# roryclear/clearcam

Measured on AMD Instinct MI355X. Metric: yolov9c_640x640_frames_per_sec, higher is better.
Workload: dtype f16; 1 GPU; YOLOv9-C f16h batch=64 640x640 frames (letterbox 640) per GPU, uint8 BGR frames resident in HBM, seeded synthetic weights, full detect path (letterbox+convs+decode+top300+NMS); batch_per_gpu=64, parallelism=one camera batch per GPU x1, no collective, batches_in_flight=3

## Files before the change

### clearcam_amd/_lib.py

```python
from __future__ import annotations

import ctypes as C
import os

_HERE = os.path.dirname(os.path.abspath(__file__))
LIB_PATH = os.path.join(_HERE, "libclearcam_hip.so")

SYMBOLS = [
    "cc_last_error", "cc_version", "cc_device_count",
    "cc_yolo_create", "cc_yolo_load", "cc_yolo_calibrate", "cc_yolo_calibration_info", "cc_gptq_round_f16", "cc_yolo_finalize", "cc_yolo_detect", "cc_yolo_set_in_flight", "cc_yolo_submit", "cc_yolo_wait",
    "cc_yolo_detect_ragged", "cc_yolo_submit_ragged", "cc_letterbox_geometry", "cc_yolo_plans_built",
    "cc_yolo_get_tensor", "cc_yolo_get_tensor_frames", "cc_yolo_nonfinite",
    "cc_yolo_last_gpu_ms", "cc_yolo_profile", "cc_yolo_profile_graph", "cc_yolo_destroy", "cc_conv2d_nhwc", "cc_conv2d_ex", "cc_route_log_take", "cc_conv_bench", "cc_dev_set", "cc_round_weights", "cc_attn_bench",
    "cc_dev_decode", "cc_dev_head_tail", "cc_dev_topk_nms", "cc_dev_blaze_post",
    "cc_dev_pool", "cc_dev_pool_choice", "cc_dev_fuse", "cc_dev_conv_src", "cc_dev_affine", "cc_dev_face_pre",
    "cc_dev_csp", "cc_dev_csp_choice", "cc_dev_stem",
    "cc_dev_attention", "cc_dev_layernorm", "cc_dev_assemble_ln", "cc_dev_patchify", "cc_dev_embed", "cc_dev_l2norm",
    "cc_clip_create", "cc_clip_load", "cc_clip_finalize", "cc_clip_encode_image", "cc_clip_encode_text",
    "cc_clip_set_in_flight", "cc_clip_submit_image", "cc_clip_wait",
    "cc_clip_last_gpu_ms", "cc_clip_destroy", "cc_crop_preprocess", "cc_cv_resize_linear_u8", "cc_cv_warp_affine_u8",
    "cc_blaze_create", "cc_blaze_load", "cc_blaze_finalize", "cc_blaze_detect", "cc_blaze_detect_batch", "cc_blaze_destroy",
    "cc_face_locate", "cc_face_align",
    "cc_face_create", "cc_face_load", "cc_face_finalize", "cc_face_embed", "cc_face_destroy",
    "cc_ocsort_create", "cc_ocsort_update", "cc_ocsort_update_many", "cc_ocsort_num_tracks", "cc_ocsort_destroy",
    "cc_index_create", "cc_index_create_ex", "cc_index_add", "cc_index_add_grouped", "cc_index_size", "cc_index_info", "cc_index_scores", "cc_index_last_path",
    "cc_index_search", "cc_index_search_groups", "cc_index_add_tracked", "cc_index_search_tracks", "cc_index_rank",
    "cc_index_add_described", "cc_index_row_info", "cc_index_rank_where", "cc_index_timeline", "cc_index_fetch_rows", "cc_index_rank_like",
    "cc_index_rank_terms", "cc_index_timeline_terms",
    "cc_index_gram", "cc_index_distinct", "cc_index_digest", "cc_index_sightings",
    "cc_index_remove_rows", "cc_index_remove_groups", "cc_index_destroy",
    "cc_watch_create", "cc_watch_set", "cc_watch_size", "cc_watch_scores", "cc_watch_match", "cc_watch_destroy",
]


class ClipConfig(C.Structure):
    _fields_ = [(n, C.c_int) for n in ("image_size", "patch", "v_width", "v_layers", "v_heads", "v_mlp",
                                       "t_ctx", "t_vocab", "t_width", "t_layers", "t_heads", "t_mlp", "embed")]


class ConvDesc(C.Structure):
    _fields_ = [(n, C.c_int) for n in ("dtype", "B", "H", "W", "Cin", "Cout", "k", "stride", "groups", "act", "pad", "Ho", "Wo",
                                       "out_f32", "out_cstride", "out_coff", "res_f32", "res_cstride", "res_coff", "variant")]


class SrcDesc(C.Structure):
    _fields_ = [("ptr", C.c_void_p)] + [(n, C.c_int) for n in ("H", "W", "cstride", "coff", "C", "shift")]


DEV_CSP_LAYERS = 3
DEV_CONV_ADOWN = 100
ROUTE_REC_INTS = 18


class FaceAlignRec(C.Structure):
    _fields_ = [("offset", C.c_int64), ("h", C.c_int32), ("w", C.c_int32),
                ("cx1", C.c_int32), ("cy1", C.c_int32), ("cw", C.c_int32), ("ch", C.c_int32),
                ("out_w", C.c_int32), ("out_h", C.c_int32), ("rot", C.c_double * 6), ("place", C.c_double * 6)]


ROW_NO_TS = -(1 << 31)
RANK_TRACKS = 1
LIKE_MAX_ROWS = 64
LIKE_EXCLUDE_ROWS, LIKE_EXCLUDE_TRACK = 2, 4
TERMS_MAX = 64
TERM_RANK, TERM_REQUIRE, TERM_REJECT = 0, 1, 2
COMBINE_MAX, COMBINE_MIN, COMBINE_SUM = 0, 1, 2
DISTINCT_MAX_DEPTH, DISTINCT_MAX_Q = 1024, 64
DIGEST_MAX_LEADERS = 1024
DIGEST_BY_COUNT, DIGEST_BY_FIRST = 0, 1
SIGHT_MAX_OBJECTS, SIGHT_MAX_GROUPS = 1024, 4096
SIGHT_SKIP_SELF = 1


class RowFilter(C.Structure):
    _fields_ = [("use_ts", C.c_int32), ("ts_min", C.c_int32), ("ts_max", C.c_int32), ("use_cls", C.c_int32), ("cls_mask", C.c_uint64 * 4)]


class Term(C.Structure):
    _fields_ = [("role", C.c_int32), ("weight", C.c_float), ("cut", C.c_float)]


class CCError(RuntimeError):
    pass


_lib = None


def lib() -> C.CDLL:
    global _lib
    if _lib is not None:
        return _lib
    if not os.path.exists(LIB_PATH):
        raise CCError(f"{LIB_PATH} not built: run `python -c 'import __graft_entry__ as g; g.build()'` "
                      "(hipcc --offload-arch=gfx950). There is no CPU fallback.")
    try:
        import torch
    except ImportError:
        pass
    L = C.CDLL(LIB_PATH)
    L.cc_last_error.restype = C.c_char_p
    vp, ip, fp, i64p = C.c_void_p, C.POINTER(C.c_int), C.POINTER(C.c_float), C.POINTER(C.c_int64)
    sig = {
        "cc_version": [],
        "cc_device_count": [ip],
        "cc_yolo_create": [C.POINTER(vp), C.c_char_p, C.c_int, C.c_int, C.c_int],
        "cc_yolo_load": [vp, C.c_char_p, vp, i64p, C.c_int],
        "cc_yolo_finalize": [vp],
        "cc_yolo_calibrate": [vp, vp, C.c_int, C.c_int, C.c_int, C.c_int],
        "cc_yolo_calibration_info": [vp, ip, ip],
        "cc_gptq_round_f16": [vp, C.c_int64, C.c_int64, vp, C.c_double, vp],
        "cc_yolo_detect": [vp, vp, C.c_int, C.c_int, C.c_int, C.c_int, C.c_int, vp, C.c_int, vp],
        "cc_yolo_set_in_flight": [vp, C.c_int],
        "cc_yolo_submit": [vp, vp, C.c_int, C.c_int, C.c_int, C.c_int, C.c_int, vp, C.c_int, vp, C.POINTER(C.c_longlong)],
        "cc_yolo_wait": [vp, C.c_longlong, vp],
        "cc_yolo_detect_ragged": [vp, vp, i64p, C.POINTER(C.c_int32), C.POINTER(C.c_int32), C.c_int, C.c_int, C.c_int, vp, C.c_int, vp],
        "cc_yolo_submit_ragged": [vp, vp, i64p, C.POINTER(C.c_int32), C.POINTER(C.c_int32), C.c_int, C.c_int, C.c_int, vp, C.c_int, vp, C.POINTER(C.c_longlong)],
        "cc_letterbox_geometry": [C.c_int, C.c_int, C.c_int, ip, ip, ip, ip],
        "cc_yolo_plans_built": [vp, ip],
        "cc_yolo_get_tensor": [vp, C.c_char_p, vp, i64p, ip],
        "cc_yolo_get_tensor_frames": [vp, C.c_char_p, C.c_int, C.c_int, vp, i64p, ip],
        "cc_yolo_nonfinite": [vp, ip],
        "cc_yolo_last_gpu_ms": [vp, fp],
        "cc_yolo_profile": [vp, C.c_int, fp, C.POINTER(C.c_double), ip],
        "cc_yolo_profile_graph": [vp, C.c_int, C.c_int, fp],
        "cc_conv2d_nhwc": [C.c_int, vp, C.c_int, C.c_int, C.c_int, C.c_int, vp, vp, C.c_int, C.c_int, C.c_int, C.c_int,
                           C.c_int, vp, C.c_int, vp],
        "cc_conv2d_ex": [C.POINTER(ConvDesc), vp, vp, vp, vp, vp, vp, ip, vp],
        "cc_route_log_take": [ip, C.c_int, ip],
        "cc_dev_decode": [vp, ip, ip, C.c_int, vp, C.c_float, vp, ip, vp],
        "cc_dev_head_tail": [C.c_int, C.c_int, vp, vp, vp, vp, vp, vp, ip, ip, C.c_int, vp, C.c_float, vp, ip, vp],
        "cc_dev_topk_nms": [vp, C.c_int, C.c_int, C.c_float, vp, C.c_int, vp, vp],
        "cc_dev_blaze_post": [vp, vp, vp, vp, C.c_int, vp, C.c_float, C.c_int, C.c_int, vp, vp, vp, vp],
        "cc_dev_pool": [C.c_int, vp, C.c_int, C.c_int, vp] + [C.c_int] * 12 + [ip, vp],
        "cc_dev_pool_choice": [C.c_int, vp, C.c_int, C.c_int, vp] + [C.c_int] * 12 + [ip],
        "cc_dev_fuse": [C.c_int, C.c_int, vp, ip, ip, ip, ip, ip, vp, C.c_int, C.c_int, C.c_int, C.c_int, C.c_int, C.c_int, vp],
        "cc_dev_conv_src": [C.POINTER(ConvDesc), C.POINTER(SrcDesc), C.POINTER(SrcDesc), vp, vp, vp, ip, vp],
        "cc_dev_affine": [C.c_int, vp, vp, vp, vp, C.c_longlong, C.c_int, vp],
        "cc_dev_face_pre": [C.c_int, vp, C.c_int, vp, C.c_int, C.c_int, vp],
        "cc_dev_csp": [C.c_int, C.c_int, C.c_int, vp, C.c_int, C.c_int, vp, C.c_int, C.c_int, C.c_int, C.c_int, C.c_int, C.POINTER(vp), C.POINTER(vp),
                       C.c_int, C.c_int, ip, vp],
        "cc_dev_csp_choice": [C.c_int] * 8 + [ip],
        "cc_dev_stem": [C.c_int, C.c_int, vp, C.c_int, i64p, C.POINTER(C.c_int32), C.POINTER(C.c_int32), C.c_int, C.c_int, C.c_int, vp, vp, C.c_int,
                        vp, C.c_int, C.c_int, ip, vp],
        "cc_dev_attention": [C.c_int, vp, C.c_int, C.c_int, C.c_int, C.c_int, C.c_float, vp, vp],
        "cc_dev_layernorm": [C.c_int, vp, C.c_longlong, vp, vp, vp, vp, C.c_int, C.c_int, C.c_int, vp],
        "cc_dev_assemble_ln": [C.c_int, vp, vp, vp, vp, vp, vp, C.c_int, C.c_int, C.c_int, vp],
        "cc_dev_patchify": [C.c_int, vp, vp, C.c_int, C.c_int, C.c_int, C.c_int, vp],
        "cc_dev_embed": [vp, C.c_int, vp, vp, vp, C.c_int, C.c_int, C.c_int, vp],
        "cc_dev_l2norm": [vp, C.c_int, C.c_int, C.c_float, vp],
        "cc_conv_bench": [C.c_int] * 11 + [fp],
        "cc_dev_set": [C.c_char_p, C.c_int],
        "cc_round_weights": [C.c_int, vp, C.c_int64, C.c_int64, C.c_int64, vp],
        "cc_attn_bench": [C.c_int] * 7 + [fp],
        "cc_clip_create": [C.POINTER(vp), C.POINTER(ClipConfig), C.c_int, C.c_int],
        "cc_clip_load": [vp, C.c_char_p, vp, i64p, C.c_int],
        "cc_clip_finalize": [vp],
        "cc_clip_encode_image": [vp, vp, C.c_int, C.c_int, vp, C.c_int, vp],
        "cc_clip_encode_text": [vp, vp, C.c_int, vp, C.c_int, vp],
        "cc_clip_set_in_flight": [vp, C.c_int],
        "cc_clip_submit_image": [vp, vp, C.c_int, C.c_int, vp, C.c_int, vp, C.POINTER(C.c_longlong)],
        "cc_clip_wait": [vp, C.c_longlong, vp],
        "cc_clip_last_gpu_ms": [vp, fp],
        "cc_crop_preprocess": [vp, vp, vp, vp, C.c_int, C.c_int, C.c_int, vp, C.c_int, vp],
        "cc_cv_resize_linear_u8": [vp, C.c_int, C.c_int, vp, C.c_int, C.c_int, C.c_int],
        "cc_cv_warp_affine_u8": [vp, C.c_int, C.c_int, vp, vp, C.c_int, C.c_int, C.c_int],
        "cc_blaze_create": [C.POINTER(vp), C.c_int, C.c_int],
        "cc_blaze_load": [vp, C.c_char_p, vp, i64p, C.c_int],
        "cc_blaze_finalize": [vp],
        "cc_blaze_detect": [vp, vp, C.c_int, C.c_int, C.c_int, C.c_int, vp, C.c_int, vp],
        "cc_blaze_detect_batch": [vp, vp, C.c_int, C.c_int, C.c_int, C.c_int, C.c_int, vp, C.c_int, vp],
        "cc_face_locate": [vp, vp, C.c_int64, vp, vp, vp, C.c_int, C.c_int, vp, vp, vp],
        "cc_face_align": [vp, C.c_int64, C.c_int, vp, C.c_int, vp, C.c_int, vp],
        "cc_face_create": [C.POINTER(vp), C.c_int, C.c_int],
        "cc_face_load": [vp, C.c_char_p, vp, i64p, C.c_int],
        "cc_face_finalize": [vp],
        "cc_face_embed": [vp, vp, C.c_int, C.c_int, C.c_int, vp, C.c_int, vp],
        "cc_ocsort_create": [C.POINTER(vp), C.c_int, C.c_int, C.c_double, C.c_int, C.c_double, C.c_int],
        "cc_ocsort_update": [vp, vp, C.c_int, C.c_double, vp, C.c_int, ip],
        "cc_ocsort_update_many": [vp, C.c_int, vp, C.c_int, C.c_double, vp, C.c_int, vp, C.c_int],
        "cc_ocsort_num_tracks": [vp, ip],
        "cc_index_create": [C.POINTER(vp), C.c_int, C.c_int64, C.c_int],
        "cc_index_create_ex": [C.POINTER(vp), C.c_int, C.c_int64, C.c_int, C.c_int],
        "cc_index_add": [vp, vp, C.c_int64, C.c_int],
        "cc_index_add_grouped": [vp, vp, C.c_int64, C.c_int, vp],
        "cc_index_add_tracked": [vp, vp, C.c_int64, C.c_int, vp, vp],
        "cc_index_info": [vp, i64p, C.POINTER(C.c_int), C.POINTER(C.c_int)],
        "cc_index_search_groups": [vp, vp, C.c_int, C.c_int, vp, C.c_int, vp, vp, C.c_int, vp],
        "cc_index_search_tracks": [vp, vp, C.c_int, C.c_int, vp, C.c_int, vp, vp, C.c_int, vp],
        "cc_index_rank": [vp, vp, C.c_int, C.c_int64, C.c_int64, C.c_float, C.c_int, vp, C.c_int, vp, vp, vp, C.c_int, vp],
        "cc_index_add_described": [vp, vp, C.c_int64, C.c_int, vp, vp, vp, vp],
        "cc_index_row_info": [vp, C.c_int64, C.c_int64, vp, vp],
        "cc_index_rank_where": [vp, vp, C.c_int, C.c_int64, C.c_int64, C.c_float, C.c_int, vp, C.c_int, C.POINTER(RowFilter), vp, vp, vp, C.c_int, vp],
        "cc_index_timeline": [vp, vp, C.c_int, C.c_float, C.c_int, vp, C.c_int, C.POINTER(RowFilter), C.c_int32, C.c_int32, C.c_int, vp, vp, C.c_int, vp],
        "cc_index_fetch_rows": [vp, i64p, C.c_int, vp, C.c_int, vp],
        "cc_index_rank_like": [vp, i64p, C.c_int, C.c_int64, C.c_int64, C.c_float, C.c_int, vp, C.c_int, C.POINTER(RowFilter), vp, vp, vp, C.c_int, vp],
        "cc_index_rank_terms": [vp, vp, C.c_int, i64p, C.c_int, C.POINTER(Term), C.c_int, C.c_int64, C.c_int64, C.c_float, C.c_int, vp, C.c_int,
                                C.POINTER(RowFilter), vp, vp, vp, vp, C.c_int, vp],
        "cc_index_timeline_terms": [vp, vp, C.c_int, i64p, C.c_int, C.POINTER(Term), C.c_int, C.c_float, C.c_int, vp, C.c_int, C.POINTER(RowFilter),
                                    C.c_int32, C.c_int32, C.c_int, vp, vp, C.c_int, vp],
        "cc_index_gram": [vp, i64p, C.c_int, vp, C.c_int, vp],
        "cc_index_distinct": [vp, vp, vp, C.c_int, C.c_int, C.c_float, C.c_int64, C.c_int64, vp, vp, vp, vp, C.c_int, vp],
        "cc_index_digest": [vp, C.c_float, C.c_int, C.c_int, vp, C.c_int, C.POINTER(RowFilter), C.c_int64, C.c_int64, vp, vp, vp, vp, vp, vp, C.c_int, vp],
        "cc_index_sightings": [vp, i64p, C.c_int, C.c_float, C.c_int, vp, C.c_int, C.POINTER(RowFilter), vp, vp, vp, vp, C.c_int, vp, C.c_int, vp],
        "cc_index_remove_rows": [vp, vp, C.c_int64, i64p],
        "cc_index_remove_groups": [vp, vp, C.c_int, i64p],
        "cc_index_size": [vp, i64p],
        "cc_index_scores": [vp, vp, C.c_int, vp, C.c_int, vp],
        "cc_index_last_path": [vp, ip],
        "cc_index_search": [vp, vp, C.c_int, C.c_int, vp, vp, C.c_int, vp],
        "cc_watch_create": [C.POINTER(vp), C.c_int, C.c_int],
        "cc_watch_set": [vp, vp, vp, vp, C.c_int],
        "cc_watch_size": [vp, ip],
        "cc_watch_scores": [vp, vp, C.c_int, C.c_int, vp, C.c_int, vp],
        "cc_watch_match": [vp, vp, C.c_int, C.c_int, vp, vp, vp, vp, C.c_int, vp],
    }
    for name, args in sig.items():
        fn = getattr(L, name)
        fn.argtypes = args
        fn.restype = C.c_int
    for name in ("cc_yolo_destroy", "cc_clip_destroy", "cc_index_destroy", "cc_ocsort_destroy", "cc_face_destroy", "cc_blaze_destroy", "cc_watch_destroy"):
        getattr(L, name).argtypes = [vp]
        getattr(L, name).restype = None
    _lib = L
    return L


def check(rc: int) -> None:
    if rc != 0:
        raise CCError(f"libclearcam_hip error {rc}: {lib().cc_last_error().decode(errors='replace')}")


def ptr(x):
    if x is None:
        return None
    if isinstance(x, int):
        return C.c_void_p(x)
    if hasattr(x, "data_ptr"):
        return C.c_void_p(x.data_ptr())
    return C.c_void_p(x.ctypes.data)
```

### clearcam_amd/csrc/conv_mfma.hip

```cpp
#include <algorithm>
#include <vector>
#include "conv_select.h"
#include "conv_tile.h"

namespace cc {

template <class T, int BM, int BN, int WM, bool SIMPLE, int CPRW, int NS, int NTH = 2 * BM>
__global__ __launch_bounds__(NTH) void conv_mfma_kernel(const ConvP p, const ConvAux a) {
  constexpr int NT = NTH, WN = NT / 64 / WM;
  constexpr int MI = BM / WM / 16, NJ = BN / WN / 16;
  constexpr int E = 16 / (int)sizeof(T);
  constexpr int BK = CPRW * E;
  constexpr int RPP = NT / CPRW;
  constexpr int XR = BM / RPP;
  constexpr int WR = BN / RPP;
  constexpr int LPS = XR + WR;
  constexpr int STAGE = (BM + BN) * CPRW;
  static_assert(BN % RPP == 0, "BN too small for this row width");
  static_assert(NS * STAGE * 16 >= BM * BN * 2, "epilogue tile must fit in the stages");
  static_assert(MI >= 1 && NJ >= 1, "bad wave layout");
  static_assert((NS - 2) * LPS < 64, "vmcnt is a 6-bit counter");
  extern __shared__ __attribute__((aligned(16))) uint4 lds[];

  const int tid = threadIdx.x, lane = tid & 63, wave = tid >> 6;
  const int M = p.B * p.Ho * p.Wo, hw = p.Ho * p.Wo;
  const unsigned lds_base = lds_addr(lds);

  int wg;
  {
    const int nwg = gridDim.x, bid = blockIdx.x;
    const int q = nwg >> 3, r = nwg & 7, xcd = bid & 7, idx = bid >> 3;
    wg = (xcd < r ? xcd * (q + 1) : r * (q + 1) + (xcd - r) * q) + idx;
  }
  const int mt_ = wg / a.nt;
  const int m0 = mt_ * BM, n0 = (wg - mt_ * a.nt) * BN;

  const int ppos = tid % CPRW, prow = tid / CPRW;
  const int chunk = ppos ^ swz<CPRW>(prow);
  const char* rowp[XR]; unsigned vmask[XR];
  const char* cur[XR]; unsigned inc[XR];
  int pb[XR], ph0[XR], pw0[XR];
#pragma unroll
  for (int i = 0; i < XR; ++i) {
    const int m = m0 + prow + RPP * i;
    if constexpr (SIMPLE) {
      if (a.is1x1) {
        rowp[i] = reinterpret_cast<const char*>(p.s0.ptr) + ((size_t)m * p.s0.cstride + p.s0.coff) * sizeof(T);
        vmask[i] = m < M ? 1u : 0u;
      } else {
        const int mm = m < M ? m : 0;
        const int b = fdiv(mm, hw, a.inv_hw), rem = mm - b * hw, ho = fdiv(rem, p.Wo, a.inv_wo), wo = rem - ho * p.Wo;
        const int h0 = ho * p.stride - p.pad, w0 = wo * p.stride - p.pad;
        unsigned hm = 0, wm = 0;
#pragma unroll
        for (int r = 0; r < 3; ++r) {
          hm |= (unsigned)(r < p.ks && (unsigned)(h0 + r) < (unsigned)p.Hin) << r;
          wm |= (unsigned)(r < p.ks && (unsigned)(w0 + r) < (unsigned)p.Win) << r;
        }
        const unsigned vm = ((hm & 1u) ? wm : 0u) | ((hm & 2u) ? wm << p.ks : 0u) | ((hm & 4u) ? wm << (2 * p.ks) : 0u);
        vmask[i] = m < M ? vm : 0u;
        rowp[i] = reinterpret_cast<const char*>(p.s0.ptr) +
                  ((((long)b * p.s0.H + h0) * p.s0.W + w0) * (long)p.s0.cstride + p.s0.coff) * (long)sizeof(T);
      }
    } else {
      if (m < M) {
        const int b = fdiv(m, hw, a.inv_hw), rem = m - b * hw, ho = fdiv(rem, p.Wo, a.inv_wo), wo = rem - ho * p.Wo;
        pb[i] = b; ph0[i] = ho * p.stride - p.pad; pw0[i] = wo * p.stride - p.pad;
      } else { pb[i] = 0; ph0[i] = -(1 << 28); pw0[i] = 0; }
    }
  }
  const char* wcur[WR]; unsigned winc[WR];
#pragma unroll
  for (int i = 0; i < WR; ++i) {
    const int n = n0 + prow + RPP * i;
    const bool ok = n < p.Cout;
    wcur[i] = ok ? reinterpret_cast<const char*>(p.w) + ((size_t)n * p.Kw + chunk * E) * sizeof(T) : reinterpret_cast<const char*>(&g_zero16);
    winc[i] = ok ? (unsigned)(BK * sizeof(T)) : 0u;
  }
  int k0 = chunk * E, kc, kr, ks_, vt;
  if (k0 < p.Cin) { kc = k0; kr = 0; ks_ = 0; vt = 0; }
  else { vt = k0 / p.Cin; kc = k0 - vt * p.Cin; const int tap = vt >> p.split; kr = tap / p.ks; ks_ = tap - kr * p.ks; }

  auto retarget = [&]() {
    const bool kok = kr < p.ks;
    const int tbit = kr * p.ks + ks_;
    const long delta = ((long)(kr * p.s0.W + ks_) * p.s0.cstride + kc) * (long)sizeof(T);
#pragma unroll
    for (int i = 0; i < XR; ++i) {
      const bool ok = kok && ((vmask[i] >> tbit) & 1u);
      cur[i] = ok ? rowp[i] + delta : reinterpret_cast<const char*>(&g_zero16);
      inc[i] = ok ? (unsigned)(BK * sizeof(T)) : 0u;
    }
  };
  if constexpr (SIMPLE) retarget();

  auto issue_loads = [&](int stage) {
    const unsigned sbase = __builtin_amdgcn_readfirstlane(lds_base + (unsigned)(stage * STAGE + wave * 64) * 16u);
    if constexpr (SIMPLE) {
#pragma unroll
      for (int i = 0; i < XR; ++i) glds16(cur[i], sbase + i * (NT * 16u));
    } else {
      const bool kok = k0 < p.Ktot;
      const bool first = kc < p.s0.C;
      const T* sp = reinterpret_cast<const T*>(first ? p.s0.ptr : p.s1.ptr);
      const int scs = first ? p.s0.cstride : p.s1.cstride, sco = first ? p.s0.coff : p.s1.coff;
      const int cc = first ? kc : kc - p.s0.C;
      const int sH = first ? p.s0.H : p.s1.H, sW = first ? p.s0.W : p.s1.W, ssh = first ? p.s0.shift : p.s1.shift;
#pragma unroll
      for (int i = 0; i < XR; ++i) {
        const int ih = ph0[i] + kr, iw = pw0[i] + ks_;
        const bool ok = kok && (unsigned)ih < (unsigned)p.Hin && (unsigned)iw < (unsigned)p.Win;
        const size_t off = ((size_t)(pb[i] * sH + (ih >> ssh)) * sW + (iw >> ssh)) * scs + sco + cc;
        glds16(ok ? static_cast<const void*>(sp + off) : static_cast<const void*>(&g_zero16), sbase + i * (NT * 16u));
      }
    }
#pragma unroll
    for (int i = 0; i < WR; ++i) glds16(wcur[i], sbase + (BM * CPRW + i * NT) * 16u);
  };
  auto advance_k = [&]() {
    k0 += BK; kc += BK;
#pragma unroll
    for (int i = 0; i < WR; ++i) wcur[i] += winc[i];
    if (kc >= p.Cin) {
      do { kc -= p.Cin; ++vt; if (next_filter_tap(vt, p.split)) { if (++ks_ == p.ks) { ks_ = 0; ++kr; } } } while (kc >= p.Cin);
      if constexpr (SIMPLE) retarget();
    } else if constexpr (SIMPLE) {
#pragma unroll
      for (int i = 0; i < XR; ++i) cur[i] += inc[i];
    }
  };

  const int wm0 = (wave % WM) * (BM / WM), wn0 = (wave / WM) * (BN / WN);
  const int fr = lane & 15, fg = lane >> 4;
  const int nkt = (p.Ktot + BK - 1) / BK;

  f32x4 acc[NJ][MI];
#pragma unroll
  for (int j = 0; j < NJ; ++j)
#pragma unroll
    for (int i = 0; i < MI; ++i) acc[j][i] = f32x4{0.f, 0.f, 0.f, 0.f};

  int issued = 0;
#pragma unroll
  for (int s = 0; s < NS - 1; ++s)
    if (s < nkt) { if (s > 0) advance_k(); issue_loads(s); ++issued; }
  int st_c = 0, st_i = NS - 1;
  for (int kt = 0; kt < nkt; ++kt) {
    const int ahead = issued - kt - 1;
    if (NS > 5 && ahead >= 4) wait_vmcnt<4 * LPS>();
    else if (NS > 4 && ahead >= 3) wait_vmcnt<3 * LPS>();
    else if (NS > 3 && ahead >= 2) wait_vmcnt<2 * LPS>();
    else if (NS > 2 && ahead >= 1) wait_vmcnt<LPS>();
    else wait_vmcnt<0>();
    __syncthreads();
    if (issued < nkt) { advance_k(); issue_loads(st_i); ++issued; if (++st_i == NS) st_i = 0; }
    const uint4* ldsX = lds + st_c * STAGE;
    const uint4* ldsW = ldsX + BM * CPRW;
    if (++st_c == NS) st_c = 0;
#pragma unroll
    for (int h = 0; h < CPRW / 4; ++h) {
      uint4 xf[MI], wf[NJ];
#pragma unroll
      for (int i = 0; i < MI; ++i) { const int row = wm0 + i * 16 + fr; xf[i] = ldsX[row * CPRW + ((h * 4 + fg) ^ swz<CPRW>(row))]; }
#pragma unroll
      for (int j = 0; j < NJ; ++j) { const int row = wn0 + j * 16 + fr; wf[j] = ldsW[row * CPRW + ((h * 4 + fg) ^ swz<CPRW>(row))]; }
#pragma unroll
      for (int j = 0; j < NJ; ++j)
#pragma unroll
        for (int i = 0; i < MI; ++i) Mma<T>::run(wf[j], xf[i], acc[j][i]);
    }
  }

  conv_epilogue<T, BM, BN, WM, MI, NJ, NT>(p, acc, n0, lds, [&](int row) { const int m = m0 + row; return m < M ? (long)m : -1L; });
}

template <class T, int TS>
__global__ __launch_bounds__(256, (TS == 256 ? 1 : 2)) void conv_big_kernel(const ConvP p, const ConvAux a) {
  constexpr int BM = TS, BN = TS, NT = 256, WM = 2, WN = 2, MI = BM / WM / 16, NJ = BN / WN / 16;
  constexpr int NF = MI + NJ, MF = MI * NJ, MPG = MF / NF;
  constexpr int E = 8, CPRW = 8, BK = 64, RPP = NT / CPRW, XR = BM / RPP, WR = BN / RPP;
  constexpr int STAGE = (BM + BN) * CPRW;
  static_assert(XR + WR == NF && MF % NF == 0 && NF % 2 == 0, "one DMA piece and MF/NF MFMAs per fragment read");
  static_assert(sizeof(T) == 2, "16-bit storage only");
  extern __shared__ __attribute__((aligned(16))) uint4 lds[];
  const int tid = threadIdx.x, lane = tid & 63, wave = tid >> 6;
  const int M = p.B * p.Ho * p.Wo, hw = p.Ho * p.Wo;
  const unsigned lds_base = lds_addr(lds);
  int wg;
  {
    const int nwg = gridDim.x, bid = blockIdx.x;
    const int q = nwg >> 3, r = nwg & 7, xcd = bid & 7, idx = bid >> 3;
    wg = (xcd < r ? xcd * (q + 1) : r * (q + 1) + (xcd - r) * q) + idx;
  }
  const int mt_ = wg / a.nt;
  const int m0 = mt_ * BM, n0 = (wg - mt_ * a.nt) * BN;

  const int ppos = tid % CPRW, prow = tid / CPRW;
  const int chunk = ppos ^ swz<CPRW>(prow);
  const char* rowp[XR]; unsigned vmask[XR];
  const char* cur[XR]; unsigned inc[XR];
#pragma unroll
  for (int i = 0; i < XR; ++i) {
    const int m = m0 + prow + RPP * i;
    if (a.is1x1) {
      rowp[i] = reinterpret_cast<const char*>(p.s0.ptr) + ((size_t)m * p.s0.cstride + p.s0.coff) * sizeof(T);
      vmask[i] = m < M ? 1u : 0u;
    } else {
      const int mm = m < M ? m : 0;
      const int b = fdiv(mm, hw, a.inv_hw), rem = mm - b * hw, ho = fdiv(rem, p.Wo, a.inv_wo), wo = rem - ho * p.Wo;
      const int h0 = ho * p.stride - p.pad, w0 = wo * p.stride - p.pad;
      unsigned hm = 0, wmk = 0;
#pragma unroll
      for (int r = 0; r < 3; ++r) {
        hm |= (unsigned)(r < p.ks && (unsigned)(h0 + r) < (unsigned)p.Hin) << r;
        wmk |= (unsigned)(r < p.ks && (unsigned)(w0 + r) < (unsigned)p.Win) << r;
      }
      const unsigned vm = ((hm & 1u) ? wmk : 0u) | ((hm & 2u) ? wmk << p.ks : 0u) | ((hm & 4u) ? wmk << (2 * p.ks) : 0u);
      vmask[i] = m < M ? vm : 0u;
      rowp[i] = reinterpret_cast<const char*>(p.s0.ptr) +
                ((((long)b * p.s0.H + h0) * p.s0.W + w0) * (long)p.s0.cstride + p.s0.coff) * (long)sizeof(T);
    }
  }
  const char* wcur[WR]; unsigned winc[WR];
#pragma unroll
  for (int i = 0; i < WR; ++i) {
    const int n = n0 + prow + RPP * i;
    const bool ok = n < p.Cout;
    wcur[i] = ok ? reinterpret_cast<const char*>(p.w) + ((size_t)n * p.Kw + chunk * E) * sizeof(T) : reinterpret_cast<const char*>(&g_zero16);
    winc[i] = ok ? (unsigned)(BK * sizeof(T)) : 0u;
  }
  int k0 = chunk * E, kc, kr, ks_, vt;
  if (k0 < p.Cin) { kc = k0; kr = 0; ks_ = 0; vt = 0; }
  else { vt = k0 / p.Cin; kc = k0 - vt * p.Cin; const int tap = vt >> p.split; kr = tap / p.ks; ks_ = tap - kr * p.ks; }
  auto retarget = [&]() {
    const bool kok = kr < p.ks;
    const int tbit = kr * p.ks + ks_;
    const long delta = ((long)(kr * p.s0.W + ks_) * p.s0.cstride + kc) * (long)sizeof(T);
#pragma unroll
    for (int i = 0; i < XR; ++i) {
      const bool ok = kok && ((vmask[i] >> tbit) & 1u);
      cur[i] = ok ? rowp[i] + delta : reinterpret_cast<const char*>(&g_zero16);
      inc[i] = ok ? (unsigned)(BK * sizeof(T)) : 0u;
    }
  };
  retarget();
  auto advance_k = [&]() {
    k0 += BK; kc += BK;
#pragma unroll
    for (int i = 0; i < WR; ++i) wcur[i] += winc[i];
    if (kc >= p.Cin) {
      do { kc -= p.Cin; ++vt; if (next_filter_tap(vt, p.split)) { if (++ks_ == p.ks) { ks_ = 0; ++kr; } } } while (kc >= p.Cin);
      retarget();
    } else {
#pragma unroll
      for (int i = 0; i < XR; ++i) cur[i] += inc[i];
    }
  };
  auto issue_piece = [&](int stage, int q) {
    const unsigned sbase = __builtin_amdgcn_readfirstlane(lds_base + (unsigned)(stage * STAGE + wave * 64) * 16u);
    if (q < XR) glds16_m0(cur[q], sbase + q * (NT * 16u));
    else glds16_m0(wcur[q - XR], sbase + (BM * CPRW + (q - XR) * NT) * 16u);
  };

  const int wm0 = (wave % WM) * (BM / WM), wn0 = (wave / WM) * (BN / WN);
  const int fr = lane & 15, fg = lane >> 4;
  const int nkt = (p.Ktot + BK - 1) / BK;
  f32x4 acc[NJ][MI];
#pragma unroll
  for (int j = 0; j < NJ; ++j)
#pragma unroll
    for (int i = 0; i < MI; ++i) acc[j][i] = f32x4{0.f, 0.f, 0.f, 0.f};

  uint4 f0[NF], f1[NF];
  auto frag = [&](int stage, int h, int q) -> uint4 {
    const int row = (q < MI ? wm0 + q * 16 : BM + wn0 + (q - MI) * 16) + fr;
    const int srow = q < MI ? row : row - BM;
    return lds[stage * STAGE + row * CPRW + ((h * 4 + fg) ^ swz<CPRW>(srow))];
  };

#pragma unroll
  for (int q = 0; q < XR + WR; ++q) issue_piece(0, q);
  if (nkt > 1) {
    advance_k();
#pragma unroll
    for (int q = 0; q < XR + WR; ++q) issue_piece(1, q);
    wait_vmcnt<XR + WR>();
  } else {
    wait_vmcnt<0>();
  }
  __syncthreads();
#pragma unroll
  for (int q = 0; q < NF; ++q) f0[q] = frag(0, 0, q);

  auto step = [&](int kt, auto more_tag, auto more2_tag) {
    constexpr bool MORE = decltype(more_tag)::value, MORE2 = decltype(more2_tag)::value;
    const int st = kt & 1;
#pragma unroll
    for (int g = 0; g < NF; ++g) {
      f1[g] = frag(st, 1, g);
#pragma unroll
      for (int u = 0; u < MPG; ++u) { const int e = g * MPG + u, j = e / MI, i = e % MI; Mma<T>::run(f0[MI + j], f0[i], acc[j][i]); }
      __builtin_amdgcn_sched_barrier(0);
    }
#pragma unroll
    for (int g = 0; g < NF / 2; ++g) {
#pragma unroll
      for (int u = 0; u < MPG; ++u) { const int e = g * MPG + u, j = e / MI, i = e % MI; Mma<T>::run(f1[MI + j], f1[i], acc[j][i]); }
      __builtin_amdgcn_sched_barrier(0);
    }
    if constexpr (MORE) {
      wait_vmcnt<0>();
      __syncthreads();
      if constexpr (MORE2) advance_k();
    }
#pragma unroll
    for (int g = NF / 2; g < NF; ++g) {
      const int q = 2 * (g - NF / 2);
      if constexpr (MORE2) { issue_piece(st, q); issue_piece(st, q + 1); }
      if constexpr (MORE) { f0[q] = frag(st ^ 1, 0, q); f0[q + 1] = frag(st ^ 1, 0, q + 1); }
#pragma unroll
      for (int u = 0; u < MPG; ++u) { const int e = g * MPG + u, j = e / MI, i = e % MI; Mma<T>::run(f1[MI + j], f1[i], acc[j][i]); }
      __builtin_amdgcn_sched_barrier(0);
    }
  };
  int kt = 0;
  for (; kt + 2 < nkt; ++kt) step(kt, std::true_type{}, std::true_type{});
  if (kt + 1 < nkt) { step(kt, std::true_type{}, std::false_type{}); ++kt; }
  step(kt, std::false_type{}, std::false_type{});
  conv_epilogue<T, BM, BN, WM, MI, NJ, NT>(p, acc, n0, lds, [&](int row) { const int m = m0 + row; return m < M ? (long)m : -1L; });
}

struct WsAux { float inv_tiles, inv_tx; int tiles, tx, total; };

template <class T, int CIN, int COUT>
__global__ __launch_bounds__(256) void conv3x3_ws_kernel(const ConvP p, const WsAux a) {
  constexpr int BM = 128, WM = 2, WN = 2, MI = 4, NJ = COUT / WN / 16;
  constexpr int E = 8, CPRW = CIN / E;
  constexpr int PW = 18, RPP = 256 / CPRW;
  constexpr int XPASS = (180 + RPP - 1) / RPP, PROWS = XPASS * RPP;
  constexpr int XP = PROWS * CPRW;
  constexpr int WROWS = 9 * COUT, WPASS = (WROWS + RPP - 1) / RPP;
  constexpr int WL = WPASS * RPP * CPRW;
  constexpr int ET = BM * COUT * 2 / 16;
  constexpr int HS = CPRW / 4;
  static_assert(sizeof(T) == 2 && (CIN == 32 || CIN == 64) && (COUT == 32 || COUT == 64), "narrow 16-bit layers only");
  extern __shared__ __attribute__((aligned(16))) uint4 lds[];
  uint4* ldsW = lds;
  uint4* ldsE = lds + WL + 2 * XP;
  const int tid = threadIdx.x, lane = tid & 63, wave = tid >> 6;
  const unsigned lds_base = lds_addr(lds);
  const int ppos = tid % CPRW, prow = tid / CPRW;

#pragma unroll
  for (int i = 0; i < WPASS; ++i) {
    const int R = prow + RPP * i;
    const int tap = R / COUT, n = R - tap * COUT;
    const int chunk = ppos ^ swz<CPRW>(R);
    const void* src = (R < WROWS && n < p.Cout) ? static_cast<const void*>(reinterpret_cast<const char*>(p.w) +
                          ((size_t)n * p.Kw + tap * CIN + chunk * E) * sizeof(T)) : static_cast<const void*>(&g_zero16);
    glds16(src, __builtin_amdgcn_readfirstlane(lds_base + (unsigned)((RPP * i) * CPRW + wave * 64) * 16u));
  }

  auto issue_patch = [&](int tile, int buf) {
    const int b = fdiv(tile, a.tiles, a.inv_tiles), trem = tile - b * a.tiles, ty = fdiv(trem, a.tx, a.inv_tx), tx = trem - ty * a.tx;
    const int h0 = ty * 8 - 1, w0 = tx * 16 - 1;
#pragma unroll
    for (int i = 0; i < XPASS; ++i) {
      const int pr = prow + RPP * i;
      const int py = pr / PW, px = pr - py * PW;
      const int ih = h0 + py, iw = w0 + px;
      const bool ok = pr < 180 && (unsigned)ih < (unsigned)p.Hin && (unsigned)iw < (unsigned)p.Win;
      const int chunk = ppos ^ swz<CPRW>(pr);
      const void* src = ok ? static_cast<const void*>(reinterpret_cast<const char*>(p.s0.ptr) +
                                 ((((long)b * p.s0.H + ih) * p.s0.W + iw) * (long)p.s0.cstride + p.s0.coff + chunk * E) * (long)sizeof(T))
                           : static_cast<const void*>(&g_zero16);
      glds16(src, __builtin_amdgcn_readfirstlane(lds_base + (unsigned)(WL + buf * XP + (RPP * i) * CPRW + wave * 64) * 16u));
    }
  };

  const int wm = wave & 1, wn0 = (wave >> 1) * (COUT / WN);
  const int fr = lane & 15, fg = lane >> 4;
  int tile = blockIdx.x, buf = 0;
  if (tile < a.total) issue_patch(tile, 0);
  for (; tile < a.total; tile += gridDim.x, buf ^= 1) {
    wait_vmcnt<0>();
    __syncthreads();
    if (tile + (int)gridDim.x < a.total) issue_patch(tile + gridDim.x, buf ^ 1);
    const uint4* ldsX = lds + WL + buf * XP;
    f32x4 acc[NJ][MI];
#pragma unroll
    for (int j = 0; j < NJ; ++j)
#pragma unroll
      for (int i = 0; i < MI; ++i) acc[j][i] = f32x4{0.f, 0.f, 0.f, 0.f};
#pragma unroll
    for (int tap = 0; tap < 9; ++tap) {
      const int r = tap / 3, sft = tap % 3;
#pragma unroll
      for (int h = 0; h < HS; ++h) {
        uint4 xf[MI], wf[NJ];
#pragma unroll
        for (int i = 0; i < MI; ++i) {
          const int row = (wm * 4 + i + r) * PW + fr + sft;
          xf[i] = ldsX[row * CPRW + ((h * 4 + fg) ^ swz<CPRW>(row))];
        }
#pragma unroll
        for (int j = 0; j < NJ; ++j) {
          const int row = tap * COUT + wn0 + j * 16 + fr;
          wf[j] = ldsW[row * CPRW + ((h * 4 + fg) ^ swz<CPRW>(row))];
        }
#pragma unroll
        for (int j = 0; j < NJ; ++j)
#pragma unroll
          for (int i = 0; i < MI; ++i) Mma<T>::run(wf[j], xf[i], acc[j][i]);
      }
    }
    const int b = fdiv(tile, a.tiles, a.inv_tiles), trem = tile - b * a.tiles, ty = fdiv(trem, a.tx, a.inv_tx), tx = trem - ty * a.tx;
    conv_epilogue<T, BM, COUT, WM, MI, NJ>(p, acc, 0, ldsE, [&](int row) {
      const int ho = ty * 8 + (row >> 4), wo = tx * 16 + (row & 15);
      return (ho < p.Ho && wo < p.Wo) ? ((long)b * p.Ho + ho) * p.Wo + wo : -1L;
    });
  }
}

template <class T> static bool supported_t(const ConvP& p) {
  const int E = 16 / (int)sizeof(T);
  auto src_ok = [&](const Src& s) { return s.C == 0 || (s.C % E == 0 && s.coff % E == 0 && s.cstride % E == 0 && ((uintptr_t)s.ptr & 15) == 0); };
  if (!src_ok(p.s0) || !src_ok(p.s1)) return false;
  if (p.Cin % E || p.Cout % 4 || p.out_coff % 4 || p.out_cstride % 4) return false;
  if (p.res && (p.res_coff % 4 || p.res_cstride % 4)) return false;
  if (p.s0.C + p.s1.C != p.Cin || p.Ktot != p.ks * p.ks * p.Cin * (p.split ? 2 : 1)) return false;
  if (p.split && (sizeof(T) != 2 || p.s0.shift < 0)) return false;
  if (p.Kw < (p.Ktot + 8 * E - 1) / (8 * E) * (8 * E)) return false;
  if ((long)p.B * p.Ho * p.Wo >= (1L << 31) || (long)p.Ho * p.Wo >= (1L << 22)) return false;
  return true;
}

bool conv_mfma_supported(int dt, const ConvP& p) {
  return dt == F32 ? supported_t<float>(p) : supported_t<f16_t>(p);
}

bool conv_persist_ok(const ConvP& p);
bool conv_tile64_legal(const ConvP& p);
void launch_conv_tile64(int dt, const ConvP& p, const ConvChoice& c, hipStream_t stream);
bool conv_wave_legal(const ConvP& p);
void launch_conv_wave(int dt, const ConvP& p, const ConvChoice& c, hipStream_t stream);
bool conv_stream_legal(const ConvP& p);
void launch_conv_stream(int dt, const ConvP& p, const ConvChoice& c, hipStream_t stream);
void launch_conv_phase(int dt, const ConvP& p, const ConvAux& a, const ConvChoice& c, hipStream_t stream);

std::atomic<int> g_stream_override{-1}, g_phase_flags_override{-1}, g_tile64_w_override{-1}, g_stream_flags_override{-1};
std::atomic<int> g_stream_abl{0}, g_tile64_abl{0};

const ConvSwitches& conv_switches() {
  static const ConvSwitches s = [] {
    auto env = [](const char* name, int dflt) { const char* e = getenv(name); return e ? atoi(e) : dflt; };
    ConvSwitches w;
    w.stream = env("CLEARCAM_STREAM", 1);
    w.stream_min_pix = env("CLEARCAM_STREAM_MIN_PIX", 200000);
    w.stream_flags = env("CLEARCAM_STREAM_FLAGS", 10);
    w.ws = env("CLEARCAM_WS", 1);
    w.small_tiles = env("CLEARCAM_SMALL_TILES", 1);
    w.small_pix = env("CLEARCAM_SMALL_PIX", 1);
    w.wave = env("CLEARCAM_WAVE", 1);
    w.tile64 = env("CLEARCAM_TILE64", 1);
    w.tile64_w = env("CLEARCAM_TILE64_W", 0);
    w.big_tile = env("CLEARCAM_BIG_TILE", 1);
    w.phase = env("CLEARCAM_PHASE", 2);
    w.phase_flags = env("CLEARCAM_PHASE_FLAGS", -1);
    return w;
  }();
  return s;
}

static bool known_variant(int v) {
  switch (v) {
    case CONV_AUTO: case CONV_DIRECT: case CONV_GENERIC: case CONV_WS: case CONV_BIG256: case CONV_BIG128: case CONV_PHASE: case CONV_WAVE:
    case CONV_SMALL: case CONV_STREAM: case CONV_TILE64: case CONV_SMALL_32_4: case CONV_SMALL_32_6: case CONV_SMALL_64_3:
    case CONV_PIX64_6: case CONV_PIX64_4: case CONV_PIX32_6: case CONV_PIX32_4: return true;
    default: return false;
  }
}

static ConvChoice generic(int bm, int bn, int wm, int cprw, int ns, bool simple) {
  ConvChoice c;
  c.bm = bm; c.bn = bn; c.wm = wm; c.cprw = cprw; c.ns = ns; c.simple = simple;
  c.nth = bm == 256 ? 512 : 256;
  return c;
}

static bool ws_legal(const ConvP& p) {
  return !p.split && p.ks == 3 && p.stride == 1 && p.pad == 1 && p.s1.C == 0 && p.s0.shift == 0 && (p.Cin == 32 || p.Cin == 64) &&
         p.Cout <= 64 && p.Cout % 8 == 0 && p.Hin == p.Ho && p.Win == p.Wo;
}
static bool ws_applicable(const ConvP& p) {
  if (!conv_switches().ws || !ws_legal(p)) return false;
  const long covered = (long)((p.Ho + 7) / 8 * 8) * ((p.Wo + 15) / 16 * 16);
  if ((long)p.Ho * p.Wo * 5 < covered * 4) return false;
  if (p.Cin == 32 && p.Cout <= 32) return true;
  const long tiles = (long)p.B * (covered / 128);
  return tiles >= 256L * 32;
}
static ConvChoice ws_choice(const ConvP& p) {
  ConvChoice c; c.kernel = ConvKernel::Ws; c.cin = p.Cin; c.cout = p.Cout > 32 ? 64 : 32;
  return c;
}

static bool choose_small(const ConvP& p, int M, bool simple, ConvChoice& c) {
  const int v = p.variant;
  const bool force = v != CONV_AUTO;
  if (!force && !conv_switches().small_tiles) return false;
  const long mt = (M + 127) / 128, b32 = mt * ((p.Cout + 31) / 32), b64 = mt * ((p.Cout + 63) / 64);
  int bn = 0;
  if (b32 <= 512) bn = 32; else if (b64 <= 512) bn = 64;
  if (force && !bn) bn = 64;
  if (!bn) return false;
  bool deep = bn == 32 && b32 <= 256;
  if (v >= CONV_SMALL_32_4 && v <= CONV_SMALL_64_3) { bn = v == CONV_SMALL_64_3 ? 64 : 32; deep = v == CONV_SMALL_32_6; }
  const long n32 = (p.Cout + 31) / 32, t32 = (long)((M + 31) / 32) * n32, t64 = (long)((M + 63) / 64) * n32;
  int pix = 0, st = 4;
  if (v == CONV_AUTO && conv_switches().small_pix) { if (t32 <= 800) { pix = 32; st = p.Ktot >= 4096 ? 6 : 4; } else if (t64 <= 512) pix = 64; }
  if (v == CONV_PIX64_6) { pix = 64; st = 6; } else if (v == CONV_PIX64_4) pix = 64; else if (v == CONV_PIX32_6) { pix = 32; st = 6; } else if (v == CONV_PIX32_4) pix = 32;
  if (pix) c = generic(pix, 32, pix == 32 ? 2 : 4, 8, st, simple);
  else if (deep) c = generic(128, 32, 4, 8, 6, simple);
  else if (bn == 32) c = generic(128, 32, 4, 8, 4, simple);
  else c = generic(128, 64, 2, 8, 3, simple);
  return true;
}

static ConvChoice phase_choice(const ConvP& p, int M, bool simple, bool two) {
  ConvChoice c; c.kernel = ConvKernel::Phase; c.bm = c.bn = 256; c.nth = 512; c.simple = simple; c.two = two;
  const int ov = g_phase_flags_override.load();
  int flags = ov >= 0 ? ov : conv_switches().phase_flags;
  const bool persist_ok = conv_persist_ok(p);
  if (flags < 0) {
    const bool is1x1 = simple && p.ks == 1 && p.stride == 1 && p.pad == 0 && p.Hin == p.Ho && p.Win == p.Wo;
    const long tiles = (long)((M + 255) / 256) * ((p.Cout + 255) / 256);
    flags = ((tiles >= 640 || (is1x1 && tiles > 256)) && persist_ok) ? 512 : 32;
  }
  const size_t xb = (size_t)p.B * p.s0.H * p.s0.W * p.s0.cstride * 2, wbytes = (size_t)p.Cout * p.Kw * 2;
  const bool buf_ok = xb < ((size_t)1 << 32) - 256 && wbytes < ((size_t)1 << 32) - 256;
  c.flags = flags;
  if ((flags & 512) && persist_ok) c.sched = PHASE_PERSIST;
  else if ((flags & 64) && buf_ok && !two) c.sched = PHASE_BUFFER;
  else c.sched = (flags & 32) ? PHASE_ONE_TILE : PHASE_SCHED0;
  return c;
}

bool conv_tile64_takes(int B, int H, int W) {
  const long per_frame = std::min((long)((H + 7) / 8) * ((W + 31) / 32), (long)((H + 15) / 16) * ((W + 15) / 16));
  return conv_switches().tile64 && (long)B * per_frame >= 256 && per_frame * 256 * 4 <= (long)H * W * 5;
}

ConvChoice choose_conv(int dt, const ConvP& p) {
  const int v = p.variant;
  CC_CHECK(known_variant(v), "conv: ConvP::variant names no kernel");
  ConvChoice c;
  if (v == CONV_DIRECT || !conv_mfma_supported(dt, p)) { c.kernel = ConvKernel::Direct; return c; }
  const int M = p.B * p.Ho * p.Wo;
  const bool simple = p.s1.C == 0 && p.s0.shift == 0 && p.ks <= 3;
  if (dt != F32) {
    const int so = g_stream_override.load(), fo = g_stream_flags_override.load();
    const int stream_on = so >= 0 ? so : conv_switches().stream;
    if (v == CONV_STREAM || (v == CONV_AUTO && stream_on && M >= conv_switches().stream_min_pix && conv_stream_legal(p))) {
      c.kernel = ConvKernel::Stream; c.cin = p.Cin; c.cout = p.Cout; c.flags = fo >= 0 ? fo : conv_switches().stream_flags;
      return c;
    }
    if (v == CONV_AUTO && ws_legal(p) && (long)((M + 127) / 128) * ((p.Cout + 31) / 32) <= 512) return ws_choice(p);
    if ((v == CONV_AUTO || v == CONV_SMALL || v >= CONV_SMALL_32_4) && choose_small(p, M, simple, c)) return c;
    if (v == CONV_TILE64 || (v == CONV_AUTO && conv_tile64_legal(p) && conv_tile64_takes(p.B, p.Ho, p.Wo))) {
      const int wo = g_tile64_w_override.load(), forced = wo >= 0 ? wo : conv_switches().tile64_w;
      const long t32 = (long)((p.Ho + 7) / 8) * ((p.Wo + 31) / 32), t16 = (long)((p.Ho + 15) / 16) * ((p.Wo + 15) / 16);
      c.kernel = ConvKernel::Tile64; c.tile64_w = (forced == 16 || (forced != 32 && t16 <= t32)) ? 16 : 32;
      return c;
    }
    const long subtiles = (long)p.B * ((p.Ho + 1) / 2) * ((p.Wo + 15) / 16);
    if (v == CONV_WAVE || (v == CONV_AUTO && conv_switches().wave && conv_wave_legal(p) && p.Cin == 64 && subtiles >= 4096)) {
      c.kernel = ConvKernel::Wave; c.cin = p.Cin; c.cout = p.Cout;
      return c;
    }
    if (v == CONV_WS || (v == CONV_AUTO && ws_applicable(p))) {
      CC_CHECK(ws_legal(p), "weights-stationary 3x3: shape not eligible");
      return ws_choice(p);
    }
  }
  auto padded = [&](int bn) { return (p.Cout + bn - 1) / bn * bn; };
  int bn = 128;
  if (padded(64) < padded(bn)) bn = 64;
  if (padded(32) < padded(bn)) bn = 32;
  if (dt != F32 && p.Cout % 256 == 0) {
    const int big = conv_switches().big_tile, phase = conv_switches().phase;
    const long tiles = (long)((M + 255) / 256) * (p.Cout / 256), rounds = (tiles + 255) / 256;
    const bool fits = p.Ktot >= 1024 && tiles >= 256 && rounds * 256 * 100 <= tiles * 112;
    if ((big > 0 && fits && !p.res && v == CONV_AUTO) || big < 0 || v == CONV_BIG256 || v == CONV_PHASE) bn = 256;
    const long t128 = (long)((M + 127) / 128) * ((p.Cout + 127) / 128);
    const double fill256 = (double)tiles / (double)(rounds * 256), fill128 = (double)t128 / (double)(((t128 + 511) / 512) * 512);
    const bool phase_rule = tiles >= 128 && fill256 * 1.2 >= fill128;
    const bool concat1 = p.s1.C > 0 && p.ks == 1 && p.stride == 1 && p.pad == 0 && p.s0.C % 64 == 0 && p.s1.C % 64 == 0;
    if ((v == CONV_AUTO || (v == CONV_PHASE && concat1)) && (simple || concat1) && p.Cin % 64 == 0 && (phase == 1 || v == CONV_PHASE || (phase != 0 && phase_rule)))
      return phase_choice(p, M, simple, concat1);
  }
  if (v == CONV_BIG128) bn = 128;
  const bool single_barrier = dt != F32 && simple;
  if (bn == 256) {
    if (single_barrier && v == CONV_PHASE) {
      CC_CHECK(p.Cin % 64 == 0 && p.Cout % 256 == 0, "eight-wave 256x256 kernel: Cin must be a multiple of 64 and Cout of 256");
      return phase_choice(p, M, simple, false);
    }
    c = generic(256, 256, 4, 8, 2, simple);
    if (single_barrier) c.kernel = ConvKernel::Big;
    return c;
  }
  if (bn == 128 && single_barrier && (p.Ktot >= 1024 || v == CONV_BIG128)) { c = generic(128, 128, 2, 8, 2, simple); c.kernel = ConvKernel::Big; return c; }
  if (bn == 32) return generic(128, 32, 4, 8, 2, simple);
  if (p.Ktot * (int)dtype_size(dt) <= 512) return generic(128, bn, 2, 4, 2, simple);
  return generic(128, bn, 2, 8, bn == 64 && dt != F32 && p.Ktot >= 2048 ? 3 : 2, simple);
}

template <class T, int BM, int BN, int WM, bool SIMPLE, int CPRW, int NS, int NTH>
static void launch_k(const ConvP& p, const ConvAux& a, hipStream_t stream) {
  constexpr size_t lds = (size_t)NS * (BM + BN) * CPRW * 16;
  const int mtiles = (p.B * p.Ho * p.Wo + BM - 1) / BM;
  ensure_max_lds(conv_mfma_kernel<T, BM, BN, WM, SIMPLE, CPRW, NS, NTH>, lds);
  note_launch(BM == 256 ? "conv_mfma_256" : (BM == 64 ? "conv_mfma_64" : (BM == 32 ? "conv_mfma_32" : "conv_mfma_128")), conv_mfma_kernel<T, BM, BN, WM, SIMPLE, CPRW, NS, NTH>, (long)mtiles * a.nt, NTH, lds);
  hipLaunchKernelGGL((conv_mfma_kernel<T, BM, BN, WM, SIMPLE, CPRW, NS, NTH>), dim3(mtiles * a.nt), dim3(NTH), lds, stream, p, a);
}

template <class T, bool SIMPLE> static void launch_generic(const ConvP& p, const ConvAux& a, const ConvChoice& c, hipStream_t stream) {
#define CC_GENERIC(BM, BN, WM, CPRW, NS, NTH) \
  if (c.bm == BM && c.bn == BN && c.wm == WM && c.cprw == CPRW && c.ns == NS && c.nth == NTH) { launch_k<T, BM, BN, WM, SIMPLE, CPRW, NS, NTH>(p, a, stream); return; }
  CC_GENERIC(128, 128, 2, 8, 2, 256)
  CC_GENERIC(128, 64, 2, 8, 2, 256)
  CC_GENERIC(128, 32, 4, 8, 2, 256)
  CC_GENERIC(128, 128, 2, 4, 2, 256)
  CC_GENERIC(128, 64, 2, 4, 2, 256)
  if constexpr (sizeof(T) == 2) {
    CC_GENERIC(256, 256, 4, 8, 2, 512)
    CC_GENERIC(128, 64, 2, 8, 3, 256)
    CC_GENERIC(128, 32, 4, 8, 4, 256)
    CC_GENERIC(128, 32, 4, 8, 6, 256)
    CC_GENERIC(64, 32, 4, 8, 4, 256)
    CC_GENERIC(64, 32, 4, 8, 6, 256)
    CC_GENERIC(32, 32, 2, 8, 4, 256)
    CC_GENERIC(32, 32, 2, 8, 6, 256)
  }
#undef CC_GENERIC
  CC_CHECK(false, "conv_mfma: no such instantiation of the generic kernel");
}

template <class T, int TS> static void launch_big(const ConvP& p, const ConvAux& a, hipStream_t stream) {
  constexpr size_t lds = (size_t)2 * (2 * TS) * 8 * 16;
  const int M = p.B * p.Ho * p.Wo;
  ensure_max_lds(conv_big_kernel<T, TS>, lds);
  note_launch(TS == 256 ? "conv_big_256" : "conv_big_128", conv_big_kernel<T, TS>, (long)((M + TS - 1) / TS) * a.nt, 256, lds);
  hipLaunchKernelGGL((conv_big_kernel<T, TS>), dim3(((M + TS - 1) / TS) * a.nt), dim3(256), lds, stream, p, a);
}

template <class T, int CIN, int COUT> static void launch_ws(const ConvP& p, hipStream_t stream) {
  constexpr int CPRW = CIN / 8, RPP = 256 / CPRW;
  constexpr int XP = (180 + RPP - 1) / RPP * RPP * CPRW, WL = (9 * COUT + RPP - 1) / RPP * RPP * CPRW;
  constexpr size_t lds = (size_t)(WL + 2 * XP + 128 * COUT * 2 / 16) * 16;
  ensure_max_lds(conv3x3_ws_kernel<T, CIN, COUT>, lds);
  const int cus = cu_count();
  WsAux a{};
  a.tx = (p.Wo + 15) / 16; a.tiles = ((p.Ho + 7) / 8) * a.tx; a.total = p.B * a.tiles;
  a.inv_tiles = 1.0f / (float)a.tiles; a.inv_tx = 1.0f / (float)a.tx;
  const int blocks_per_cu = (int)(160 * 1024 / lds);
  note_launch("conv3x3_ws", conv3x3_ws_kernel<T, CIN, COUT>, (long)a.total, 256, lds, std::min(a.total, cus * std::max(1, blocks_per_cu)));
  hipLaunchKernelGGL((conv3x3_ws_kernel<T, CIN, COUT>), dim3(std::min(a.total, cus * std::max(1, blocks_per_cu))), dim3(256), lds, stream, p, a);
}

template <class T> static void launch_t(const ConvP& p, const ConvAux& a, const ConvChoice& c, hipStream_t stream) {
  if constexpr (sizeof(T) == 2) {
    if (c.kernel == ConvKernel::Ws) {
      if (c.cin == 64) { if (c.cout == 64) launch_ws<T, 64, 64>(p, stream); else launch_ws<T, 64, 32>(p, stream); }
      else { if (c.cout == 64) launch_ws<T, 32, 64>(p, stream); else launch_ws<T, 32, 32>(p, stream); }
      return;
    }
    if (c.kernel == ConvKernel::Big) { if (c.bm == 256) launch_big<T, 256>(p, a, stream); else launch_big<T, 128>(p, a, stream); return; }
  }
  CC_CHECK(c.kernel == ConvKernel::Generic, "conv_mfma: kernel not available for this storage type");
  if (c.simple) launch_generic<T, true>(p, a, c, stream); else launch_generic<T, false>(p, a, c, stream);
}

std::atomic<int> g_route_log{0};
static std::mutex g_route_mutex;
static std::vector<int> g_route_recs;

void route_log_append(const ConvP& p, const ConvChoice& c) {
  const int sym_ho = (p.Hin + 2 * p.pad - p.ks) / p.stride + 1, sym_wo = (p.Win + 2 * p.pad - p.ks) / p.stride + 1;
  const int rec[ROUTE_REC_INTS] = {(int)c.kernel, c.sched, c.bm, c.bn, p.ks, p.stride, (p.Ho > sym_ho || p.Wo > sym_wo) ? 1 : 0, p.act,
                                   p.res ? (p.res_f32 ? 2 : 1) : 0, p.out_f32 ? 1 : 0,
                                   (p.Cout % 8 == 0 && p.out_coff % 8 == 0 && p.out_cstride % 8 == 0) ? 1 : 0,
                                   p.B, p.Hin, p.Win, p.Cin, p.Cout, p.Ho, p.Wo};
  std::lock_guard<std::mutex> lock(g_route_mutex);
  g_route_recs.insert(g_route_recs.end(), rec, rec + ROUTE_REC_INTS);
}

int route_log_take(int* recs, int cap) {
  std::lock_guard<std::mutex> lock(g_route_mutex);
  const int n = (int)(g_route_recs.size() / ROUTE_REC_INTS), take = std::min(n, std::max(cap, 0));
  if (recs && take > 0) std::copy(g_route_recs.begin(), g_route_recs.begin() + (size_t)take * ROUTE_REC_INTS, recs);
  g_route_recs.erase(g_route_recs.begin(), g_route_recs.begin() + (size_t)take * ROUTE_REC_INTS);
  return n;
}

void launch_conv_mfma(int dt, const ConvP& p, hipStream_t stream) { launch_conv_chosen(dt, p, stream, nullptr); }

void launch_conv_chosen(int dt, const ConvP& p, hipStream_t stream, ConvChoice* chosen) {
  const ConvChoice c = choose_conv(dt, p);
  if (chosen) *chosen = c;
  if (g_route_log.load(std::memory_order_relaxed)) route_log_append(p, c);
  ConvAux a{};
  a.nt = (p.Cout + c.bn - 1) / c.bn;
  a.inv_hw = 1.0f / (float)(p.Ho * p.Wo); a.inv_wo = 1.0f / (float)p.Wo;
  a.is1x1 = c.simple && p.ks == 1 && p.stride == 1 && p.pad == 0 && p.Hin == p.Ho && p.Win == p.Wo;
  a.two = c.two;
  switch (c.kernel) {
    case ConvKernel::Direct: launch_conv_direct(dt, p, stream); return;
    case ConvKernel::Stream: launch_conv_stream(dt, p, c, stream); return;
    case ConvKernel::Tile64: launch_conv_tile64(dt, p, c, stream); return;
    case ConvKernel::Wave: launch_conv_wave(dt, p, c, stream); return;
    case ConvKernel::Phase: launch_conv_phase(dt, p, a, c, stream); break;
    default:
      if (dt == F32) launch_t<float>(p, a, c, stream);
      else if (dt == F16) launch_t<f16_t>(p, a, c, stream);
      else launch_t<bf16_t>(p, a, c, stream);
  }
  CC_HIP(hipGetLastError());
}

void launch_conv(int dt, const ConvP& p, hipStream_t stream) {
  if (p.s0.shift < 0) launch_conv_adown(dt, p, stream);
  else launch_conv_mfma(dt, p, stream);
}

}
```

### clearcam_amd/csrc/conv_persist.hip

```cpp
#include "conv_tile.h"

namespace cc {

typedef __attribute__((ext_vector_type(16))) float f32x16;

template <class T> struct Mma32;
template <> struct Mma32<bf16_t> {
  static __device__ __forceinline__ void run(const uint4& a, const uint4& b, f32x16& acc) {
    acc = __builtin_amdgcn_mfma_f32_32x32x16_bf16(__builtin_bit_cast(bf16x8, a), __builtin_bit_cast(bf16x8, b), acc, 0, 0, 0);
  }
};
template <> struct Mma32<f16_t> {
  static __device__ __forceinline__ void run(const uint4& a, const uint4& b, f32x16& acc) {
    acc = __builtin_amdgcn_mfma_f32_32x32x16_f16(__builtin_bit_cast(f16x8, a), __builtin_bit_cast(f16x8, b), acc, 0, 0, 0);
  }
};

template <class T, int ACT> __device__ __forceinline__ float act_bias(float osc, float x, float b, float slope) {
  float v = activate<T, ACT>(__builtin_fmaf(x, osc, b));
  if constexpr (ACT == 3) v = v > 0.f ? v : slope * v;
  return v;
}

template <class T, int MM, int ABL = 0>
__global__ __launch_bounds__(512) void conv_persist_kernel(const ConvP p, const ConvAux a) {
  constexpr int BM = 256, BN = 256, NT = 512;
  constexpr int E = 8, CPRW = 8, BK = 64, RPP = NT / CPRW, XR = BM / RPP;
  constexpr int STAGE = (BM + BN) * CPRW;
  constexpr unsigned SB = STAGE * 16u;
  static_assert(sizeof(T) == 2, "16-bit storage");
  extern __shared__ __attribute__((aligned(16))) uint4 lds[];
  const int tid = threadIdx.x, lane = tid & 63;
  const int wave = __builtin_amdgcn_readfirstlane(tid >> 6);
  const int grp = wave >> 2, wq = wave & 3;
  const int M = p.B * p.Ho * p.Wo, hw = p.Ho * p.Wo;
  const unsigned lds_base = lds_addr(lds);
  const int ntiles = a.ntiles;
  const int ppos = tid % CPRW, prow = tid / CPRW;
  const int chunk = ppos ^ swz<CPRW>(prow);
  struct RowInfo { const char* ptr; unsigned long long aux; };
  RowInfo* rinfo = reinterpret_cast<RowInfo*>(lds + 2 * STAGE) + tid * XR;
  const char* cur[XR]; unsigned inc[XR];
  const char* wptr = nullptr;
  const size_t wpass = (size_t)RPP * p.Kw * sizeof(T);
  int kc = 0, vt = 0, pt = 0, wt = 0, m0 = 0, n0 = 0;
  const int nkt = (p.Ktot + BK - 1) / BK;
  const float osc = out_scale(p);

  auto retarget = [&]() {
    const int tap = vt >> p.split;
    const int kr = a.two ? 0 : tap / p.ks, ks_ = a.two ? 0 : tap - kr * p.ks;
    const long delta = ((long)(kr * p.s0.W + ks_) * p.s0.cstride + kc + chunk * E) * (long)sizeof(T);
#pragma unroll
    for (int i = 0; i < XR; ++i) {
      const RowInfo ri = rinfo[i];
      const bool ok = a.two ? ri.ptr != nullptr : (bool)((ri.aux >> tap) & 1u);
      const char* src = (a.two && (vt & 1)) ? reinterpret_cast<const char*>(ri.aux) : ri.ptr;
      cur[i] = ok ? src + delta : reinterpret_cast<const char*>(&g_zero16);
      inc[i] = ok ? (unsigned)(BK * sizeof(T)) : 0u;
    }
  };
  auto setup_tile = [&](int vb) {
    int tid_o = tid;
    asm volatile("" : "+v"(tid_o));
    const int prow = tid_o / CPRW;
    const int q = ntiles >> 3, r = ntiles & 7, xcd = vb & 7, idx = vb >> 3;
    const int wg = (xcd < r ? xcd * (q + 1) : r * (q + 1) + (xcd - r) * q) + idx;
    const int mt_ = wg / a.nt;
    m0 = mt_ * BM; n0 = (wg - mt_ * a.nt) * BN;
#pragma unroll
    for (int i = 0; i < XR; ++i) {
      const int m = m0 + prow + RPP * i;
      RowInfo ri;
      if (a.two) {
        const int mm = m < M ? m : 0;
        const int b = fdiv(mm, hw, a.inv_hw), rem = mm - b * hw, ho = fdiv(rem, p.Wo, a.inv_wo), wo = rem - ho * p.Wo;
        const long i0 = ((long)b * p.s0.H + (ho >> p.s0.shift)) * p.s0.W + (wo >> p.s0.shift);
        const long i1 = ((long)b * p.s1.H + (ho >> p.s1.shift)) * p.s1.W + (wo >> p.s1.shift);
        ri.ptr = m < M ? reinterpret_cast<const char*>(p.s0.ptr) + (i0 * p.s0.cstride + p.s0.coff) * (long)sizeof(T) : nullptr;
        ri.aux = (unsigned long long)(reinterpret_cast<const char*>(p.s1.ptr) + (i1 * p.s1.cstride + p.s1.coff) * (long)sizeof(T));
      } else if (a.is1x1) {
        ri.ptr = reinterpret_cast<const char*>(p.s0.ptr) + ((size_t)m * p.s0.cstride + p.s0.coff) * sizeof(T);
        ri.aux = m < M ? 1u : 0u;
      } else {
        const int mm = m < M ? m : 0;
        const int b = fdiv(mm, hw, a.inv_hw), rem = mm - b * hw, ho = fdiv(rem, p.Wo, a.inv_wo), wo = rem - ho * p.Wo;
        const int h0 = ho * p.stride - p.pad, w0 = wo * p.stride - p.pad;
        unsigned hm = 0, wmk = 0;
#pragma unroll
        for (int rr = 0; rr < 3; ++rr) {
          hm |= (unsigned)(rr < p.ks && (unsigned)(h0 + rr) < (unsigned)p.Hin) << rr;
          wmk |= (unsigned)(rr < p.ks && (unsigned)(w0 + rr) < (unsigned)p.Win) << rr;
        }
        const unsigned vm = ((hm & 1u) ? wmk : 0u) | ((hm & 2u) ? wmk << p.ks : 0u) | ((hm & 4u) ? wmk << (2 * p.ks) : 0u);
        ri.aux = m < M ? vm : 0u;
        ri.ptr = reinterpret_cast<const char*>(p.s0.ptr) +
                 ((((long)b * p.s0.H + h0) * p.s0.W + w0) * (long)p.s0.cstride + p.s0.coff) * (long)sizeof(T);
      }
      rinfo[i] = ri;
    }
    wptr = reinterpret_cast<const char*>(p.w) + ((size_t)(n0 + prow) * p.Kw + chunk * E) * sizeof(T);
    kc = 0; vt = 0; pt = 0; wt = 0;
    retarget();
  };
  auto advance_p = [&]() {
    kc += BK;
    if (kc == (a.two ? ((vt & 1) ? p.s1.C : p.s0.C) : p.Cin)) { kc = 0; ++vt; retarget(); }
    else {
#pragma unroll
      for (int i = 0; i < XR; ++i) cur[i] += inc[i];
    }
  };
  const unsigned wave_lds = __builtin_amdgcn_readfirstlane(lds_base + (unsigned)(wave * 64) * 16u);
  bool in_loop = false;
  auto issue_p = [&](unsigned stage_bytes, int h) {
    if constexpr (ABL & 1) { if (in_loop) return; }
    const unsigned sb = wave_lds + stage_bytes;
    glds16_m0(cur[2 * h], sb + (2 * h) * (NT * 16u)); glds16_m0(cur[2 * h + 1], sb + (2 * h + 1) * (NT * 16u));
  };
  auto issue_w = [&](unsigned stage_bytes, int h) {
    if constexpr (ABL & 1) { if (in_loop) return; }
    const unsigned sb = wave_lds + stage_bytes + (unsigned)(BM * CPRW) * 16u;
    glds16_m0(wptr + (2 * h) * wpass, sb + (2 * h) * (NT * 16u)); glds16_m0(wptr + (2 * h + 1) * wpass, sb + (2 * h + 1) * (NT * 16u));
  };
  auto step_w = [&]() { if (wt + 1 < nkt) { wptr += BK * sizeof(T); ++wt; } };
  auto step_p = [&]() { if (pt + 1 < nkt) { advance_p(); ++pt; } };
  auto first_pieces = [&]() {
    issue_p(0, 0); issue_p(0, 1); step_p();
    issue_w(0, 0); issue_w(0, 1); step_w();
    issue_w(SB, 0); issue_w(SB, 1); step_w();
  };

  constexpr int NA = MM ? 4 : 2;
  const char* ldsb = reinterpret_cast<const char*>(lds);
  const char* pb[NA]; const char* wbp[NA];
  {
    const int fr = MM ? (lane & 31) : (lane & 15), fh = MM ? (lane >> 5) : (lane >> 4), sw = (fr >> 1) & 7;
#pragma unroll
    for (int s = 0; s < NA; ++s) {
      const int ch = MM ? (2 * s + fh) : (4 * s + fh);
      pb[s] = ldsb + (grp * 128 + fr) * 128 + ((ch ^ sw) * 16);
      wbp[s] = ldsb + (BM + wq * 64 + fr) * 128 + ((ch ^ sw) * 16);
    }
  }
  uint4 pa[8], wb[4], wb1[4];
  f32x4 acc[MM ? 1 : 4][MM ? 1 : 8];
  f32x16 acc32[MM ? 2 : 1][MM ? 4 : 1];
  auto zero_acc = [&]() {
    if constexpr (MM == 0) {
#pragma unroll
      for (int j = 0; j < 4; ++j)
#pragma unroll
        for (int i = 0; i < 8; ++i) acc[j][i] = f32x4{0.f, 0.f, 0.f, 0.f};
    } else {
#pragma unroll
      for (int j = 0; j < 2; ++j)
#pragma unroll
        for (int i = 0; i < 4; ++i)
#pragma unroll
          for (int e = 0; e < 16; ++e) acc32[j][i][e] = 0.f;
    }
  };
  auto read_p = [&](unsigned so, int ps) {
    if constexpr (ABL & 2) { if (in_loop) return; }
    if constexpr (MM == 0) {
#pragma unroll
      for (int kh = 0; kh < 2; ++kh)
#pragma unroll
        for (int i = 0; i < 4; ++i) pa[kh * 4 + i] = *reinterpret_cast<const uint4*>(pb[kh] + so + (ps * 64 + i * 16) * 128);
    } else {
#pragma unroll
      for (int s = 0; s < 4; ++s)
#pragma unroll
        for (int i = 0; i < 2; ++i) pa[s * 2 + i] = *reinterpret_cast<const uint4*>(pb[s] + so + (ps * 64 + i * 32) * 128);
    }
  };
  auto read_w = [&](unsigned so, int ws, uint4 (&dst)[4]) {
    if constexpr (ABL & 2) { if (in_loop) return; }
    if constexpr (MM == 0) {
#pragma unroll
      for (int kh = 0; kh < 2; ++kh)
#pragma unroll
        for (int j = 0; j < 2; ++j) dst[kh * 2 + j] = *reinterpret_cast<const uint4*>(wbp[kh] + so + (ws * 32 + j * 16) * 128);
    } else {
#pragma unroll
      for (int s = 0; s < 4; ++s) dst[s] = *reinterpret_cast<const uint4*>(wbp[s] + so + (ws * 32) * 128);
    }
  };
  auto mma_w = [&](int ps, int ws, const uint4 (&wv)[4]) {
    if constexpr (ABL & 4) {
#pragma unroll
      for (int i = 0; i < 8; ++i) asm volatile("" :: "v"(pa[i].x), "v"(pa[i].y), "v"(pa[i].z), "v"(pa[i].w));
#pragma unroll
      for (int i = 0; i < 4; ++i) asm volatile("" :: "v"(wv[i].x), "v"(wv[i].y), "v"(wv[i].z), "v"(wv[i].w));
      return;
    }
    __builtin_amdgcn_s_setprio(1);
    if constexpr (MM == 0) {
#pragma unroll
      for (int kh = 0; kh < 2; ++kh)
#pragma unroll
        for (int j = 0; j < 2; ++j)
#pragma unroll
          for (int i = 0; i < 4; ++i) Mma<T>::run(wv[kh * 2 + j], pa[kh * 4 + i], acc[ws * 2 + j][ps * 4 + i]);
    } else {
#pragma unroll
      for (int s = 0; s < 4; ++s)
#pragma unroll
        for (int i = 0; i < 2; ++i) Mma32<T>::run(wv[s], pa[s * 2 + i], acc32[ws][ps * 2 + i]);
    }
    __builtin_amdgcn_s_setprio(0);
  };
  auto sync = [&]() {
    __builtin_amdgcn_sched_barrier(0);
    if constexpr (!(ABL & 8)) __builtin_amdgcn_s_barrier();
    __builtin_amdgcn_sched_barrier(0);
  };

  char* stg = reinterpret_cast<char*>(lds) + SB + wave * 4096;
  auto epilogue16 = [&](auto act_tag, int em0, int en0, const float4 (&bq)[8], bool full) {
    constexpr int ACT = decltype(act_tag)::value;
    int lane = tid & 63;
    asm volatile("" : "+v"(lane));
    const int nb = en0 + wq * 64;
    T* outp = reinterpret_cast<T*>(p.out) + p.out_coff + nb;
    const int spix = lane >> 3, schunk = lane & 7;
    const char* rdp = stg + spix * 128 + ((schunk ^ (spix & 7)) * 16);
    if constexpr (MM == 0) {
      const int fr = lane & 15, fg = lane >> 4;
      float4 b4[4], s4[4];
#pragma unroll
      for (int j = 0; j < 4; ++j) {
        b4[j] = bq[j];
        if constexpr (ACT == 3) s4[j] = *reinterpret_cast<const float4*>(p.slope + nb + j * 16 + fg * 4); else s4[j] = make_float4(0.f, 0.f, 0.f, 0.f);
      }
#pragma unroll
      for (int r = 0; r < 4; ++r) {
#pragma unroll
        for (int ib = 0; ib < 2; ++ib)
#pragma unroll
          for (int j = 0; j < 4; ++j) {
            const f32x4 av = acc[j][2 * r + ib];
            float v0 = act_bias<T, ACT>(osc, av[0], b4[j].x, s4[j].x), v1 = act_bias<T, ACT>(osc, av[1], b4[j].y, s4[j].y);
            float v2 = act_bias<T, ACT>(osc, av[2], b4[j].z, s4[j].z), v3 = act_bias<T, ACT>(osc, av[3], b4[j].w, s4[j].w);
            if constexpr (ACT == 4) { v0 = fmaxf(v0, 0.f); v1 = fmaxf(v1, 0.f); v2 = fmaxf(v2, 0.f); v3 = fmaxf(v3, 0.f); }
            const int row = ib * 16 + fr, cl = j * 2 + (fg >> 1);
            *reinterpret_cast<uint2*>(stg + row * 128 + ((cl ^ (row & 7)) * 16) + (fg & 1) * 8) = make_uint2(pack2<T>(v0, v1), pack2<T>(v2, v3));
          }
        asm volatile("" ::: "memory");
#pragma unroll
        for (int t = 0; t < 4; ++t) {
          const uint4 v = *reinterpret_cast<const uint4*>(rdp + t * 1024);
          const int m = em0 + grp * 128 + r * 32 + t * 8 + spix;
          if constexpr (ABL & 32) asm volatile("" :: "v"(v.x), "v"(v.y), "v"(v.z), "v"(v.w));
          else if (full || m < M) *reinterpret_cast<uint4*>(outp + (size_t)m * p.out_cstride + schunk * 8) = v;
        }
        asm volatile("" ::: "memory");
      }
    } else {
      const int fr = lane & 31, fh = lane >> 5;
      float4 b4[2][4], s4[2][4];
#pragma unroll
      for (int ws = 0; ws < 2; ++ws)
#pragma unroll
        for (int q = 0; q < 4; ++q) {
          const int n = nb + ws * 32 + q * 8 + fh * 4;
          b4[ws][q] = bq[ws * 4 + q];
          if constexpr (ACT == 3) s4[ws][q] = *reinterpret_cast<const float4*>(p.slope + n); else s4[ws][q] = make_float4(0.f, 0.f, 0.f, 0.f);
        }
#pragma unroll
      for (int r = 0; r < 4; ++r) {
#pragma unroll
        for (int ws = 0; ws < 2; ++ws)
#pragma unroll
          for (int q = 0; q < 4; ++q) {
            const f32x16 av = acc32[ws][r];
            float v0 = act_bias<T, ACT>(osc, av[4 * q + 0], b4[ws][q].x, s4[ws][q].x), v1 = act_bias<T, ACT>(osc, av[4 * q + 1], b4[ws][q].y, s4[ws][q].y);
            float v2 = act_bias<T, ACT>(osc, av[4 * q + 2], b4[ws][q].z, s4[ws][q].z), v3 = act_bias<T, ACT>(osc, av[4 * q + 3], b4[ws][q].w, s4[ws][q].w);
            if constexpr (ACT == 4) { v0 = fmaxf(v0, 0.f); v1 = fmaxf(v1, 0.f); v2 = fmaxf(v2, 0.f); v3 = fmaxf(v3, 0.f); }
            const int cl = ws * 4 + q;
            *reinterpret_cast<uint2*>(stg + fr * 128 + ((cl ^ (fr & 7)) * 16) + fh * 8) = make_uint2(pack2<T>(v0, v1), pack2<T>(v2, v3));
          }
        asm volatile("" ::: "memory");
#pragma unroll
        for (int t = 0; t < 4; ++t) {
          const uint4 v = *reinterpret_cast<const uint4*>(rdp + t * 1024);
          const int m = em0 + grp * 128 + r * 32 + t * 8 + spix;
          if constexpr (ABL & 32) asm volatile("" :: "v"(v.x), "v"(v.y), "v"(v.z), "v"(v.w));
          else if (full || m < M) *reinterpret_cast<uint4*>(outp + (size_t)m * p.out_cstride + schunk * 8) = v;
        }
        asm volatile("" ::: "memory");
      }
    }
  };
  auto epilogue32 = [&](auto act_tag, int em0, int en0, const float4 (&bq)[8], bool full) {
    constexpr int ACT = decltype(act_tag)::value;
    int lane = tid & 63;
    asm volatile("" : "+v"(lane));
    const int nb = en0 + wq * 64;
    const int spix = lane >> 4, schunk = lane & 15;
    const int n = nb + schunk * 4;
    const int mbase = em0 + grp * 128 + spix;
    auto load_res = [&](int k, float (&rv)[4][4]) {
      if (!p.res) return;
#pragma unroll
      for (int t = 0; t < 4; ++t) {
        const int m = mbase + k * 16 + t * 4;
        if (full || m < M) {
          const size_t ri = (size_t)m * p.res_cstride + p.res_coff + n;
          if (p.res_f32) load4<float>(p.res, ri, rv[t]); else load4<T>(p.res, ri, rv[t]);
        }
      }
    };
    auto finish = [&](int k, const float (&rv)[4][4]) {
      asm volatile("" ::: "memory");
#pragma unroll
      for (int t = 0; t < 4; ++t) {
        const int pr = t * 4 + spix;
        const float4 v = *reinterpret_cast<const float4*>(stg + pr * 256 + ((schunk ^ (pr & 15)) * 16));
        const int m = mbase + k * 16 + t * 4;
        if (full || m < M) {
          float o[4] = {v.x, v.y, v.z, v.w};
          if (p.res) {
#pragma unroll
            for (int e = 0; e < 4; ++e) o[e] = rv[t][e] + o[e];
          }
          if constexpr (ACT == 4) {
#pragma unroll
            for (int e = 0; e < 4; ++e) o[e] = fmaxf(o[e], 0.f);
          }
          const size_t oi = (size_t)m * p.out_cstride + p.out_coff + n;
          if (p.out_f32) store4<float>(p.out, oi, o); else store4<T>(p.out, oi, o);
        }
      }
      asm volatile("" ::: "memory");
    };
    float4 b4[8], s4[8];
#pragma unroll
    for (int k = 0; k < 8; ++k) {
      b4[k] = bq[k];
      s4[k] = make_float4(0.f, 0.f, 0.f, 0.f);
      if constexpr (ACT == 3) {
        if (MM == 0) { if (k < 4) s4[k] = *reinterpret_cast<const float4*>(p.slope + nb + k * 16 + (lane >> 4) * 4); }
        else s4[k] = *reinterpret_cast<const float4*>(p.slope + nb + (k >> 2) * 32 + (k & 3) * 8 + (lane >> 5) * 4);
      }
    }
    auto stage = [&](int k) {
      if constexpr (MM == 0) {
        const int fr = lane & 15, fg = lane >> 4;
#pragma unroll
        for (int j = 0; j < 4; ++j) {
          const f32x4 av = acc[j][k];
          const int cl = j * 4 + fg;
          *reinterpret_cast<float4*>(stg + fr * 256 + ((cl ^ (fr & 15)) * 16)) =
              make_float4(act_bias<T, ACT>(osc, av[0], b4[j].x, s4[j].x), act_bias<T, ACT>(osc, av[1], b4[j].y, s4[j].y),
                          act_bias<T, ACT>(osc, av[2], b4[j].z, s4[j].z), act_bias<T, ACT>(osc, av[3], b4[j].w, s4[j].w));
        }
      } else {
        const int fr = lane & 31, fh = lane >> 5, r = k >> 1, half = k & 1;
        if ((fr >> 4) == half) {
          const int row = fr & 15;
#pragma unroll
          for (int ws = 0; ws < 2; ++ws)
#pragma unroll
            for (int q = 0; q < 4; ++q) {
              const f32x16 av = acc32[ws][r];
              const float4 b = b4[ws * 4 + q], sl = s4[ws * 4 + q];
              const int cl = ws * 8 + q * 2 + fh;
              *reinterpret_cast<float4*>(stg + row * 256 + ((cl ^ (row & 15)) * 16)) =
                  make_float4(act_bias<T, ACT>(osc, av[4 * q + 0], b.x, sl.x), act_bias<T, ACT>(osc, av[4 * q + 1], b.y, sl.y),
                              act_bias<T, ACT>(osc, av[4 * q + 2], b.z, sl.z), act_bias<T, ACT>(osc, av[4 * q + 3], b.w, sl.w));
            }
        }
      }
    };
    float ra[4][4] = {}, rb[4][4] = {};
    load_res(0, ra);
#pragma unroll
    for (int k = 0; k < 8; k += 2) {
      stage(k);
      load_res(k + 1, rb);
      finish(k, ra);
      stage(k + 1);
      if (k + 2 < 8) load_res(k + 2, ra);
      finish(k + 1, rb);
    }
  };
  const bool staged16 = !p.res && !p.out_f32 && (p.out_coff % 8 == 0) && (p.out_cstride % 8 == 0);
  const bool rows32 = (p.out_f32 ? (p.out_coff % 4 == 0 && p.out_cstride % 4 == 0) : (p.out_coff % 4 == 0 && p.out_cstride % 4 == 0)) &&
                      (!p.res || (p.res_coff % 4 == 0 && p.res_cstride % 4 == 0));
  (void)rows32;
  auto load_bias = [&](int en0, float4 (&bq)[8]) {
    int lane = tid & 63;
    asm volatile("" : "+v"(lane));
    const int nb = en0 + wq * 64;
#pragma unroll
    for (int k = 0; k < 8; ++k) bq[k] = make_float4(0.f, 0.f, 0.f, 0.f);
    if (p.bias) {
      if constexpr (MM == 0) {
#pragma unroll
        for (int j = 0; j < 4; ++j) bq[j] = *reinterpret_cast<const float4*>(p.bias + nb + j * 16 + (lane >> 4) * 4);
      } else {
#pragma unroll
        for (int k = 0; k < 8; ++k) bq[k] = *reinterpret_cast<const float4*>(p.bias + nb + (k >> 2) * 32 + (k & 3) * 8 + (lane >> 5) * 4);
      }
    }
  };
  auto epilogue = [&](int em0, int en0, const float4 (&bq)[8], bool full) {
    if (staged16) {
      if (p.act == 1) epilogue16(std::integral_constant<int, 1>{}, em0, en0, bq, full);
      else if (p.act == 2) epilogue16(std::integral_constant<int, 2>{}, em0, en0, bq, full);
      else if (p.act == 3) epilogue16(std::integral_constant<int, 3>{}, em0, en0, bq, full);
      else if (p.act == 4) epilogue16(std::integral_constant<int, 4>{}, em0, en0, bq, full);
      else epilogue16(std::integral_constant<int, 0>{}, em0, en0, bq, full);
    } else {
      if (p.act == 1) epilogue32(std::integral_constant<int, 1>{}, em0, en0, bq, full);
      else if (p.act == 2) epilogue32(std::integral_constant<int, 2>{}, em0, en0, bq, full);
      else if (p.act == 3) epilogue32(std::integral_constant<int, 3>{}, em0, en0, bq, full);
      else if (p.act == 4) epilogue32(std::integral_constant<int, 4>{}, em0, en0, bq, full);
      else epilogue32(std::integral_constant<int, 0>{}, em0, en0, bq, full);
    }
  };

  int vb = blockIdx.x;
  setup_tile(vb);
  first_pieces();
  for (; vb < ntiles; vb += gridDim.x) {
    zero_acc();
    wait_vmcnt<0>();
    __builtin_amdgcn_s_barrier();
    if (grp == 1) __builtin_amdgcn_s_barrier();
    __builtin_amdgcn_sched_barrier(0);
    if constexpr (ABL & 2) { read_w(0, 0, wb); read_w(0, 1, wb1); read_p(0, 0); }
    in_loop = true;
    for (int t = 0; t < nkt; ++t) {
      const unsigned so = (t & 1) ? SB : 0u, no = SB - so;
      read_w(so, 0, wb); read_p(so, 0);
      issue_p(no, 0);
      sync(); mma_w(0, 0, wb); sync();
      read_w(so, 1, wb1);
      issue_p(no, 1); step_p();
      sync(); mma_w(0, 1, wb1); sync();
      read_p(so, 1);
      sync(); mma_w(1, 1, wb1); sync();
      issue_w(so, 0); issue_w(so, 1); step_w();
      wait_vmcnt<4>();
      sync(); mma_w(1, 0, wb); sync();
    }
    in_loop = false;
    wait_vmcnt<0>();
    if (grp == 0) __builtin_amdgcn_s_barrier();
    __builtin_amdgcn_sched_barrier(0);
    const int em0 = m0, en0 = n0;
    float4 bq[8];
    load_bias(en0, bq);
    __builtin_amdgcn_sched_barrier(0);
    if (vb + (int)gridDim.x < ntiles) { setup_tile(vb + gridDim.x); if constexpr (!(ABL & 64)) first_pieces(); }
    __builtin_amdgcn_sched_barrier(0);
    const bool full = em0 + BM <= M;
    if constexpr (!(ABL & 16)) epilogue(em0, en0, bq, full);
    else {
      if constexpr (MM == 0) {
#pragma unroll
        for (int j = 0; j < 4; ++j)
#pragma unroll
          for (int i = 0; i < 8; ++i) asm volatile("" :: "v"(acc[j][i]));
      } else {
#pragma unroll
        for (int j = 0; j < 2; ++j)
#pragma unroll
          for (int i = 0; i < 4; ++i) asm volatile("" :: "v"(acc32[j][i]));
      }
    }
    __builtin_amdgcn_sched_barrier(0);
  }
}

bool conv_persist_ok(const ConvP& p) {
  if (p.Cout % 256) return false;
  if (p.res || p.out_f32) {
    if (p.out_coff % 4 || p.out_cstride % 4) return false;
    if (p.res && (p.res_coff % 4 || p.res_cstride % 4)) return false;
  } else if (p.out_coff % 8 || p.out_cstride % 8) return false;
  return true;
}

template <class T, int MM, int ABL = 0> static void launch_persist_t(const ConvP& p, const ConvAux& a, int M, hipStream_t stream) {
  constexpr size_t lds = (size_t)2 * 512 * 8 * 16 + 512 * 4 * 16;
  ensure_max_lds(conv_persist_kernel<T, MM, ABL>, lds);
  const int cus = cu_count();
  ConvAux b = a;
  b.ntiles = ((M + 255) / 256) * a.nt;
  note_launch("conv_persist", conv_persist_kernel<T, MM, ABL>, (long)b.ntiles, 512, lds, std::min(b.ntiles, cus));
  hipLaunchKernelGGL((conv_persist_kernel<T, MM, ABL>), dim3(std::min(b.ntiles, cus)), dim3(512), lds, stream, p, b);
}

void launch_conv_persist(int dt, int mm, int abl, const ConvP& p, const ConvAux& a, int M, hipStream_t stream) {
#ifdef CC_PERSIST_ABLATIONS
  if (abl && dt == BF16 && !mm) {
    switch (abl) {
      case 1: launch_persist_t<bf16_t, 0, 1>(p, a, M, stream); return;
      case 2: launch_persist_t<bf16_t, 0, 3>(p, a, M, stream); return;
      case 3: launch_persist_t<bf16_t, 0, 4>(p, a, M, stream); return;
      case 4: launch_persist_t<bf16_t, 0, 16>(p, a, M, stream); return;
      case 5: launch_persist_t<bf16_t, 0, 11>(p, a, M, stream); return;
      case 6: launch_persist_t<bf16_t, 0, 27>(p, a, M, stream); return;
      case 7: launch_persist_t<bf16_t, 0, 32>(p, a, M, stream); return;
      case 8: launch_persist_t<bf16_t, 0, 64>(p, a, M, stream); return;
      case 9: launch_persist_t<bf16_t, 0, 96>(p, a, M, stream); return;
      case 10: launch_persist_t<bf16_t, 0, 75>(p, a, M, stream); return;
      default: break;
    }
  }
  if (mm) { if (dt == F16) launch_persist_t<f16_t, 1>(p, a, M, stream); else launch_persist_t<bf16_t, 1>(p, a, M, stream); return; }
#endif
  (void)abl; (void)mm;
  if (dt == F16) launch_persist_t<f16_t, 0>(p, a, M, stream); else launch_persist_t<bf16_t, 0>(p, a, M, stream);
}

}
```

### clearcam_amd/csrc/conv_phase.hip

```cpp
#include "conv_select.h"
#include "conv_tile.h"

namespace cc {

typedef int srd_t __attribute__((ext_vector_type(4)));
__device__ __forceinline__ srd_t make_srd(const void* base, unsigned bytes) {
  const unsigned long long b = (unsigned long long)base;
  srd_t r;
  r[0] = __builtin_amdgcn_readfirstlane((int)(b & 0xffffffffu));
  r[1] = __builtin_amdgcn_readfirstlane((int)((b >> 32) & 0xffffu));
  r[2] = __builtin_amdgcn_readfirstlane((int)bytes);
  r[3] = 0x00020000;
  return r;
}
__device__ __forceinline__ void bdma16(unsigned voff, srd_t srd, unsigned lds_wave_byte_addr) {
  asm volatile("s_mov_b32 m0, %2\n\ts_nop 0\n\tbuffer_load_dwordx4 %0, %1, 0 offen lds" : : "v"(voff), "s"(srd), "s"(lds_wave_byte_addr) : "memory", "m0");
}

template <class T, int SCHED>
__global__ __launch_bounds__(512) void conv_phase_kernel(const ConvP p, const ConvAux a) {
  constexpr int BM = 256, BN = 256, NT = 512, MI = 8, NJ = 4;
  constexpr int E = 8, CPRW = 8, BK = 64, RPP = NT / CPRW, XR = BM / RPP, WR = BN / RPP;
  constexpr int STAGE = (BM + BN) * CPRW;
  static_assert(sizeof(T) == 2 && XR == 4 && WR == 4, "16-bit storage, four DMA passes per operand");
  extern __shared__ __attribute__((aligned(16))) uint4 lds[];
  const int tid = threadIdx.x, lane = tid & 63, wave = tid >> 6;
  const int grp = wave >> 2, wq = wave & 3;
  const int M = p.B * p.Ho * p.Wo, hw = p.Ho * p.Wo;
  const unsigned lds_base = lds_addr(lds);
  int wg;
  {
    const int nwg = gridDim.x, bid = blockIdx.x;
    const int q = nwg >> 3, r = nwg & 7, xcd = bid & 7, idx = bid >> 3;
    wg = (xcd < r ? xcd * (q + 1) : r * (q + 1) + (xcd - r) * q) + idx;
  }
  const int mt_ = wg / a.nt;
  const int m0 = mt_ * BM, n0 = (wg - mt_ * a.nt) * BN;

  const int ppos = tid % CPRW, prow = tid / CPRW;
  const int chunk = ppos ^ swz<CPRW>(prow);
  constexpr bool BUF = SCHED == 2;
  struct RowInfo { const char* ptr; unsigned long long aux; };
  RowInfo* rinfo = reinterpret_cast<RowInfo*>(lds + 2 * STAGE) + tid * XR;
  const char* cur[XR]; unsigned inc[XR];
  unsigned cur32[XR];
  const srd_t srd_x = make_srd(p.s0.ptr, (unsigned)a.x_bytes), srd_w = make_srd(p.w, (unsigned)a.w_bytes);
#pragma unroll
  for (int i = 0; i < XR; ++i) {
    const int m = m0 + prow + RPP * i;
    RowInfo ri;
    if (a.two) {
      const int mm = m < M ? m : 0;
      const int b = fdiv(mm, hw, a.inv_hw), rem = mm - b * hw, ho = fdiv(rem, p.Wo, a.inv_wo), wo = rem - ho * p.Wo;
      const long i0 = ((long)b * p.s0.H + (ho >> p.s0.shift)) * p.s0.W + (wo >> p.s0.shift);
      const long i1 = ((long)b * p.s1.H + (ho >> p.s1.shift)) * p.s1.W + (wo >> p.s1.shift);
      ri.ptr = m < M ? reinterpret_cast<const char*>(p.s0.ptr) + (i0 * p.s0.cstride + p.s0.coff) * (long)sizeof(T) : nullptr;
      ri.aux = (unsigned long long)(reinterpret_cast<const char*>(p.s1.ptr) + (i1 * p.s1.cstride + p.s1.coff) * (long)sizeof(T));
    } else if (a.is1x1) {
      ri.ptr = reinterpret_cast<const char*>(p.s0.ptr) + ((size_t)m * p.s0.cstride + p.s0.coff) * sizeof(T);
      ri.aux = m < M ? 1u : 0u;
    } else {
      const int mm = m < M ? m : 0;
      const int b = fdiv(mm, hw, a.inv_hw), rem = mm - b * hw, ho = fdiv(rem, p.Wo, a.inv_wo), wo = rem - ho * p.Wo;
      const int h0 = ho * p.stride - p.pad, w0 = wo * p.stride - p.pad;
      unsigned hm = 0, wmk = 0;
#pragma unroll
      for (int r = 0; r < 3; ++r) {
        hm |= (unsigned)(r < p.ks && (unsigned)(h0 + r) < (unsigned)p.Hin) << r;
        wmk |= (unsigned)(r < p.ks && (unsigned)(w0 + r) < (unsigned)p.Win) << r;
      }
      const unsigned vm = ((hm & 1u) ? wmk : 0u) | ((hm & 2u) ? wmk << p.ks : 0u) | ((hm & 4u) ? wmk << (2 * p.ks) : 0u);
      ri.aux = m < M ? vm : 0u;
      ri.ptr = reinterpret_cast<const char*>(p.s0.ptr) +
               ((((long)b * p.s0.H + h0) * p.s0.W + w0) * (long)p.s0.cstride + p.s0.coff) * (long)sizeof(T);
    }
    rinfo[i] = ri;
  }
  const char* wptr = reinterpret_cast<const char*>(p.w) + ((size_t)(n0 + prow) * p.Kw + chunk * E) * sizeof(T);
  const size_t wpass = (size_t)RPP * p.Kw * sizeof(T);
  int kc = 0, vt = 0;
  auto retarget = [&]() {
    const int tap = vt >> p.split;
    const int kr = a.two ? 0 : tap / p.ks, ks_ = a.two ? 0 : tap - kr * p.ks;
    const long delta = ((long)(kr * p.s0.W + ks_) * p.s0.cstride + kc + chunk * E) * (long)sizeof(T);
#pragma unroll
    for (int i = 0; i < XR; ++i) {
      const RowInfo ri = rinfo[i];
      const bool ok = a.two ? ri.ptr != nullptr : (bool)((ri.aux >> tap) & 1u);
      const char* src = (a.two && (vt & 1)) ? reinterpret_cast<const char*>(ri.aux) : ri.ptr;
      if constexpr (BUF) cur32[i] = ok ? (unsigned)((src + delta) - reinterpret_cast<const char*>(p.s0.ptr)) : 0xffffffffu;
      else cur[i] = ok ? src + delta : reinterpret_cast<const char*>(&g_zero16);
      inc[i] = ok ? (unsigned)(BK * sizeof(T)) : 0u;
    }
  };
  retarget();
  auto advance_p = [&]() {
    kc += BK;
    if (kc == (a.two ? ((vt & 1) ? p.s1.C : p.s0.C) : p.Cin)) { kc = 0; ++vt; retarget(); }
    else {
#pragma unroll
      for (int i = 0; i < XR; ++i) { if constexpr (BUF) cur32[i] += inc[i]; else cur[i] += inc[i]; }
    }
  };
  const unsigned wave_lds = __builtin_amdgcn_readfirstlane(lds_base + (unsigned)(wave * 64) * 16u);
  auto issue_p = [&](unsigned stage_bytes, int h) {
    const unsigned sb = wave_lds + stage_bytes;
    if constexpr (BUF) { bdma16(cur32[2 * h], srd_x, sb + (2 * h) * (NT * 16u)); bdma16(cur32[2 * h + 1], srd_x, sb + (2 * h + 1) * (NT * 16u)); }
    else { glds16_m0(cur[2 * h], sb + (2 * h) * (NT * 16u)); glds16_m0(cur[2 * h + 1], sb + (2 * h + 1) * (NT * 16u)); }
  };
  auto issue_w = [&](unsigned stage_bytes, int h) {
    const unsigned sb = wave_lds + stage_bytes + (unsigned)(BM * CPRW) * 16u;
    if constexpr (BUF) {
      const unsigned w32 = (unsigned)(wptr - reinterpret_cast<const char*>(p.w));
      bdma16(w32 + (2 * h) * (unsigned)wpass, srd_w, sb + (2 * h) * (NT * 16u)); bdma16(w32 + (2 * h + 1) * (unsigned)wpass, srd_w, sb + (2 * h + 1) * (NT * 16u));
    } else { glds16_m0(wptr + (2 * h) * wpass, sb + (2 * h) * (NT * 16u)); glds16_m0(wptr + (2 * h + 1) * wpass, sb + (2 * h + 1) * (NT * 16u)); }
  };

  const int fr = lane & 15, fg = lane >> 4;
  const int nkt = (p.Ktot + BK - 1) / BK;
  f32x4 acc[NJ][MI];
#pragma unroll
  for (int j = 0; j < NJ; ++j)
#pragma unroll
    for (int i = 0; i < MI; ++i) acc[j][i] = f32x4{0.f, 0.f, 0.f, 0.f};
  uint4 pa[8], wb[4];
  uint4 wb1[4];
  const int sw = (fr >> 1) & 7;
  const char* ldsb = reinterpret_cast<const char*>(lds);
  const char* pb[2] = {ldsb + (grp * 128 + fr) * 128 + ((fg ^ sw) * 16), ldsb + (grp * 128 + fr) * 128 + (((4 + fg) ^ sw) * 16)};
  const char* wbp[2] = {ldsb + (BM + wq * 64 + fr) * 128 + ((fg ^ sw) * 16), ldsb + (BM + wq * 64 + fr) * 128 + (((4 + fg) ^ sw) * 16)};
  auto read_p = [&](unsigned so, int ps) {
#pragma unroll
    for (int kh = 0; kh < 2; ++kh)
#pragma unroll
      for (int i = 0; i < 4; ++i)
        pa[kh * 4 + i] = *reinterpret_cast<const uint4*>(pb[kh] + so + (ps * 64 + i * 16) * 128);
  };
  auto read_w = [&](unsigned so, int ws) {
#pragma unroll
    for (int kh = 0; kh < 2; ++kh)
#pragma unroll
      for (int j = 0; j < 2; ++j)
        wb[kh * 2 + j] = *reinterpret_cast<const uint4*>(wbp[kh] + so + (ws * 32 + j * 16) * 128);
  };
  auto mma_w = [&](int ps, int ws, const uint4 (&wv)[4], auto&& mid) {
    __builtin_amdgcn_s_setprio(1);
#pragma unroll
    for (int kh = 0; kh < 2; ++kh)
#pragma unroll
      for (int j = 0; j < 2; ++j) {
#pragma unroll
        for (int i = 0; i < 4; ++i) Mma<T>::run(wv[kh * 2 + j], pa[kh * 4 + i], acc[ws * 2 + j][ps * 4 + i]);
        if (kh == 0 && j == 0) { __builtin_amdgcn_sched_barrier(0); mid(); __builtin_amdgcn_sched_barrier(0); }
      }
    __builtin_amdgcn_s_setprio(0);
  };
  auto mma = [&](int ps, int ws, auto&& mid) { mma_w(ps, ws, wb, mid); };
  auto read_w1 = [&](unsigned so) {
#pragma unroll
    for (int kh = 0; kh < 2; ++kh)
#pragma unroll
      for (int j = 0; j < 2; ++j)
        wb1[kh * 2 + j] = *reinterpret_cast<const uint4*>(wbp[kh] + so + (32 + j * 16) * 128);
  };
  auto end_read = [&]() {
    __builtin_amdgcn_sched_barrier(0);
    asm volatile("s_waitcnt lgkmcnt(0)" ::: "memory");
    __builtin_amdgcn_sched_barrier(0);
    __builtin_amdgcn_s_barrier();
    __builtin_amdgcn_sched_barrier(0);
  };
  auto end_mma = [&]() {
    __builtin_amdgcn_sched_barrier(0);
    __builtin_amdgcn_s_barrier();
    __builtin_amdgcn_sched_barrier(0);
  };

  int pt = 0, wt = 0;
  auto step_w = [&]() { if (wt + 1 < nkt) { wptr += BK * sizeof(T); ++wt; } };
  auto step_p = [&]() { if (pt + 1 < nkt) { advance_p(); ++pt; } };
  constexpr unsigned SB = STAGE * 16u;
  auto nothing = [] {};
  if constexpr (SCHED >= 1) {
    auto sync = [&]() { __builtin_amdgcn_sched_barrier(0); __builtin_amdgcn_s_barrier(); __builtin_amdgcn_sched_barrier(0); };
    issue_p(0, 0); issue_p(0, 1); step_p();
    issue_w(0, 0); issue_w(0, 1); step_w();
    issue_w(SB, 0); issue_w(SB, 1); step_w();
    wait_vmcnt<4>();
    __builtin_amdgcn_s_barrier();
    if (grp == 1) __builtin_amdgcn_s_barrier();
    __builtin_amdgcn_sched_barrier(0);
    for (int t = 0; t < nkt; ++t) {
      const unsigned so = (t & 1) ? SB : 0u, no = SB - so;
      read_w(so, 0); read_p(so, 0);
      issue_p(no, 0);
      sync(); mma_w(0, 0, wb, nothing); sync();
      read_w1(so);
      issue_p(no, 1); step_p();
      sync(); mma_w(0, 1, wb1, nothing); sync();
      read_p(so, 1);
      sync(); mma_w(1, 1, wb1, nothing); sync();
      issue_w(so, 0); issue_w(so, 1); step_w();
      wait_vmcnt<4>();
      sync(); mma_w(1, 0, wb, nothing); sync();
    }
  } else {
  issue_p(0, 0); issue_p(0, 1); step_p();
  issue_w(0, 0); issue_w(0, 1); step_w();
  issue_p(SB, 0);
  wait_vmcnt<2>();
  __builtin_amdgcn_s_barrier();
  if (grp == 1) __builtin_amdgcn_s_barrier();
  __builtin_amdgcn_sched_barrier(0);
  if (a.flags & 24) {
    read_w(0, 0); read_p(0, 0);
    for (int t = 0; t < nkt; ++t) {
      const unsigned so = (t & 1) ? SB : 0u;
      if (a.flags & 16) { read_w(so, 0); read_p(so, 0); }
      end_read(); mma(0, 0, nothing); end_mma();
      if (a.flags & 16) read_w(so, 1);
      end_read(); mma(0, 1, nothing); end_mma();
      if (a.flags & 16) read_p(so, 1);
      end_read(); mma(1, 1, nothing); end_mma();
      if (a.flags & 16) read_w(so, 0);
      end_read(); mma(1, 0, nothing); end_mma();
    }
  } else
  for (int t = 0; t < nkt; ++t) {
    const unsigned so = (t & 1) ? SB : 0u, no = SB - so;
    read_w(so, 0); read_p(so, 0);
    issue_p(no, 1); step_p();
    end_read(); mma(0, 0, nothing); end_mma();
    read_w(so, 1);
    issue_w(no, 0);
    end_read(); mma(0, 1, nothing); end_mma();
    read_p(so, 1);
    issue_w(no, 1); step_w();
    end_read(); mma(1, 1, nothing); end_mma();
    read_w(so, 0);
    issue_p(so, 0);
    wait_vmcnt<2>();
    end_read(); mma(1, 0, nothing); end_mma();
  }
  }
  wait_vmcnt<0>();
  if (grp == 0) __builtin_amdgcn_s_barrier();
  conv_epilogue<T, BM, BN, 2, MI, NJ, NT, true>(p, acc, n0, lds, [&](int row) { const int m = m0 + row; return m < M ? (long)m : -1L; });
}

bool conv_persist_ok(const ConvP& p);
void launch_conv_persist(int dt, int mm, int abl, const ConvP& p, const ConvAux& a, int M, hipStream_t stream);
template <class T, int SCHED> static void launch_phase_k(const ConvP& p, const ConvAux& a, hipStream_t stream) {
  constexpr size_t lds = (size_t)2 * 512 * 8 * 16 + 512 * 4 * 16;
  const long tiles = (long)((p.B * p.Ho * p.Wo + 255) / 256) * a.nt;
  ensure_max_lds(conv_phase_kernel<T, SCHED>, lds);
  note_launch("conv_phase", conv_phase_kernel<T, SCHED>, tiles, 512, lds);
  hipLaunchKernelGGL((conv_phase_kernel<T, SCHED>), dim3(tiles), dim3(512), lds, stream, p, a);
}

template <class T> static void launch_phase(const ConvP& p, const ConvAux& a, const ConvChoice& c, hipStream_t stream) {
  ConvAux b = a; b.flags = c.flags;
  b.x_bytes = (unsigned)((size_t)p.B * p.s0.H * p.s0.W * p.s0.cstride * sizeof(T)); b.w_bytes = (unsigned)((size_t)p.Cout * p.Kw * sizeof(T));
  switch (c.sched) {
    case PHASE_PERSIST: launch_conv_persist(TypeTag<T>::dt, (c.flags & 1024) ? 1 : 0, (c.flags >> 12) & 15, p, b, p.B * p.Ho * p.Wo, stream); break;
    case PHASE_BUFFER: launch_phase_k<T, 2>(p, b, stream); break;
    case PHASE_ONE_TILE: launch_phase_k<T, 1>(p, b, stream); break;
    default: launch_phase_k<T, 0>(p, b, stream);
  }
}

void launch_conv_phase(int dt, const ConvP& p, const ConvAux& a, const ConvChoice& c, hipStream_t stream) {
  CC_CHECK(dt != F32, "eight-wave 256x256 kernel: 16-bit storage only");
  if (dt == F16) launch_phase<f16_t>(p, a, c, stream);
  else launch_phase<bf16_t>(p, a, c, stream);
}

}
```

### clearcam_amd/csrc/conv_select.h

```cpp
#pragma once
#include <atomic>
#include "common.h"

namespace cc {

enum ConvVariant : int {
  CONV_AUTO = 0,
  CONV_DIRECT = 1,
  CONV_GENERIC = 2,
  CONV_WS = 4,
  CONV_BIG256 = 5,
  CONV_BIG128 = 6,
  CONV_PHASE = 7,
  CONV_WAVE = 8,
  CONV_SMALL = 9,
  CONV_STREAM = 10,
  CONV_TILE64 = 12,
  CONV_SMALL_32_4 = 91,
  CONV_SMALL_32_6 = 92,
  CONV_SMALL_64_3 = 93,
  CONV_PIX64_6 = 94,
  CONV_PIX64_4 = 95,
  CONV_PIX32_6 = 96,
  CONV_PIX32_4 = 97,
};

enum class ConvKernel : int { Direct, Generic, Big, Phase, Ws, Wave, Tile64, Stream };

enum { PHASE_SCHED0 = 0, PHASE_ONE_TILE = 1, PHASE_BUFFER = 2, PHASE_PERSIST = 3 };

struct ConvChoice {
  ConvKernel kernel = ConvKernel::Generic;
  int bm = 128, bn = 128, wm = 2, cprw = 8, ns = 2, nth = 256;
  bool simple = false;
  int sched = 0;
  bool two = false;
  int flags = 0;
  int tile64_w = 32;
  int cin = 0, cout = 0;
};

ConvChoice choose_conv(int dt, const ConvP& p);

bool conv_tile64_takes(int B, int H, int W);

void launch_conv_chosen(int dt, const ConvP& p, hipStream_t stream, ConvChoice* chosen);

constexpr int ROUTE_REC_INTS = 18;
extern std::atomic<int> g_route_log;
void route_log_append(const ConvP& p, const ConvChoice& c);
int route_log_take(int* recs, int cap);

struct ConvSwitches {
  int stream, stream_min_pix, stream_flags;
  int ws, small_tiles, small_pix, wave;
  int tile64, tile64_w;
  int big_tile, phase, phase_flags;
};
const ConvSwitches& conv_switches();

extern std::atomic<int> g_stream_override, g_phase_flags_override, g_tile64_w_override, g_stream_flags_override;
extern std::atomic<int> g_stream_abl, g_tile64_abl;

}
```

### clearcam_amd/csrc/conv_tile.h

```cpp
#pragma once
#include <algorithm>
#include <type_traits>
#include "kernels.h"
#include "mfma.h"

namespace cc {

static __device__ const uint4 g_zero16 = {0u, 0u, 0u, 0u};

struct ConvAux {
  float inv_hw, inv_wo;
  int nt;
  int is1x1;
  int flags;
  unsigned x_bytes, w_bytes;
  int ntiles;
  int two;
};

__device__ __forceinline__ float out_scale(const ConvP& p) { return p.split ? p.oscale : 1.0f; }
__device__ __forceinline__ bool next_filter_tap(int vt, int split) { return !(vt & split); }

template <class T, int ACT> __device__ __forceinline__ float activate(float x) {
  if constexpr (ACT == 1) {
    if constexpr (sizeof(T) == 4) return x / (1.0f + expf(-x));
    else return x * __builtin_amdgcn_rcpf(1.0f + __builtin_amdgcn_exp2f(x * -1.4426950408889634f));
  } else if constexpr (ACT == 2) {
    const float u = 0.7978845608028654f * (x + 0.044715f * x * x * x);
    if constexpr (sizeof(T) == 4) return 0.5f * x * (1.0f + tanhf(u));
    else {
      const float t = x * x;
      const float z = x * __builtin_fmaf(t, -0.044715f * 2.0f * 0.7978845608028654f * 1.4426950408889634f, -2.0f * 0.7978845608028654f * 1.4426950408889634f);
      return x * __builtin_amdgcn_rcpf(1.0f + __builtin_amdgcn_exp2f(z));
    }
  } else return x;
}
template <class T> __device__ __forceinline__ float activate_rt(float x, int act) {
  return act == 1 ? activate<T, 1>(x) : (act == 2 ? activate<T, 2>(x) : x);
}

template <class T> __device__ __forceinline__ void store4(void* base, size_t idx, const float (&v)[4]) {
  if constexpr (sizeof(T) == 4) {
    *reinterpret_cast<float4*>(reinterpret_cast<float*>(base) + idx) = make_float4(v[0], v[1], v[2], v[3]);
  } else {
    *reinterpret_cast<uint2*>(reinterpret_cast<T*>(base) + idx) = make_uint2(pack2<T>(v[0], v[1]), pack2<T>(v[2], v[3]));
  }
}
template <class T> __device__ __forceinline__ void load4(const void* base, size_t idx, float (&v)[4]) {
  if constexpr (sizeof(T) == 4) {
    const float4 f = *reinterpret_cast<const float4*>(reinterpret_cast<const float*>(base) + idx);
    v[0] = f.x; v[1] = f.y; v[2] = f.z; v[3] = f.w;
  } else {
    uint2 u = *reinterpret_cast<const uint2*>(reinterpret_cast<const T*>(base) + idx);
    const T* t = reinterpret_cast<const T*>(&u);
    for (int i = 0; i < 4; ++i) v[i] = to_f32<T>(t[i]);
  }
}

__device__ __forceinline__ void glds16(const void* src, unsigned lds_wave_byte_addr) {
  unsigned keep;
  asm volatile("s_mov_b32 %0, m0\n\ts_mov_b32 m0, %2\n\ts_nop 0\n\tglobal_load_lds_dwordx4 %1, off\n\ts_mov_b32 m0, %0"
               : "=&s"(keep) : "v"(src), "s"(lds_wave_byte_addr) : "memory");
}
__device__ __forceinline__ void glds16_m0(const void* src, unsigned lds_wave_byte_addr) {
  asm volatile("s_mov_b32 m0, %1\n\ts_nop 0\n\tglobal_load_lds_dwordx4 %0, off" : : "v"(src), "s"(lds_wave_byte_addr) : "memory", "m0");
}
__device__ __forceinline__ unsigned lds_addr(const void* p) {
  return (unsigned)(size_t)(__attribute__((address_space(3))) const void*)p;
}
__device__ __forceinline__ int fdiv(int n, int d, float inv) {
  int q = (int)((float)n * inv);
  const int r = n - q * d;
  q += (r >= d) - (r < 0);
  return q;
}

template <int CPRW> __device__ __forceinline__ int swz(int row) {
  if constexpr (CPRW == 8) return (row >> 1) & 7;
  else return (-(row >> 2)) & 3;
}
template <int N> __device__ __forceinline__ void wait_vmcnt() { asm volatile("s_waitcnt vmcnt(%0)" ::"n"(N) : "memory"); }

template <class T, int ACT, int BN, int MI, int NJ>
__device__ __forceinline__ void stage_tile(const ConvP& p, const f32x4 (&acc)[NJ][MI], char* tilep, int n0, int wm0, int wn0, int fr, int fg) {
  constexpr int ROWB = BN * 2, CPR = BN / 8;
  auto rowswz = [](int row) { if constexpr (CPR <= 16) return row / (16 / CPR); else return row * (CPR / 16); };
  const float osc = out_scale(p);
#pragma unroll
  for (int j = 0; j < NJ; ++j) {
    const int nl = wn0 + j * 16 + fg * 4, n = n0 + nl;
    float4 b4 = make_float4(0.f, 0.f, 0.f, 0.f), s4 = make_float4(0.f, 0.f, 0.f, 0.f);
    if (p.bias && n < p.Cout) b4 = *reinterpret_cast<const float4*>(p.bias + n);
    if constexpr (ACT == 3) { if (n < p.Cout) s4 = *reinterpret_cast<const float4*>(p.slope + n); }
#pragma unroll
    for (int i = 0; i < MI; ++i) {
      const f32x4 av = acc[j][i];
      float v0 = activate<T, ACT>(__builtin_fmaf(av[0], osc, b4.x)), v1 = activate<T, ACT>(__builtin_fmaf(av[1], osc, b4.y));
      float v2 = activate<T, ACT>(__builtin_fmaf(av[2], osc, b4.z)), v3 = activate<T, ACT>(__builtin_fmaf(av[3], osc, b4.w));
      if constexpr (ACT == 3) { v0 = v0 > 0.f ? v0 : s4.x * v0; v1 = v1 > 0.f ? v1 : s4.y * v1; v2 = v2 > 0.f ? v2 : s4.z * v2; v3 = v3 > 0.f ? v3 : s4.w * v3; }
      if constexpr (ACT == 4) { v0 = fmaxf(v0, 0.f); v1 = fmaxf(v1, 0.f); v2 = fmaxf(v2, 0.f); v3 = fmaxf(v3, 0.f); }
      const int row = wm0 + i * 16 + fr;
      const int ch = (nl >> 3) ^ (rowswz(row) & (CPR - 1));
      *reinterpret_cast<uint2*>(tilep + row * ROWB + ch * 16 + (nl & 4) * 2) = make_uint2(pack2<T>(v0, v1), pack2<T>(v2, v3));
    }
  }
}

template <class T, int ACT, int MI, int NJ>
__device__ __forceinline__ void direct_tile(const ConvP& p, const f32x4 (&acc)[NJ][MI], const long (&mrow)[MI], int nbase) {
  const float osc = out_scale(p);
#pragma unroll
  for (int j = 0; j < NJ; ++j) {
    const int n = nbase + j * 16;
    const bool nok = n < p.Cout;
    float bv[4] = {0.f, 0.f, 0.f, 0.f}, sv[4] = {0.f, 0.f, 0.f, 0.f};
    if (p.bias && nok) { const float4 b4 = *reinterpret_cast<const float4*>(p.bias + n); bv[0] = b4.x; bv[1] = b4.y; bv[2] = b4.z; bv[3] = b4.w; }
    if constexpr (ACT == 3) { if (nok) { const float4 s4 = *reinterpret_cast<const float4*>(p.slope + n); sv[0] = s4.x; sv[1] = s4.y; sv[2] = s4.z; sv[3] = s4.w; } }
#pragma unroll
    for (int i = 0; i < MI; ++i) {
      const f32x4 av = acc[j][i];
      const long m = mrow[i];
      if (nok && m >= 0) {
        float v[4];
#pragma unroll
        for (int e = 0; e < 4; ++e) {
          v[e] = activate<T, ACT>(__builtin_fmaf(av[e], osc, bv[e]));
          if constexpr (ACT == 3) v[e] = v[e] > 0.f ? v[e] : sv[e] * v[e];
        }
        if (p.res) {
          float rv[4];
          const size_t ri = (size_t)m * p.res_cstride + p.res_coff + n;
          if (p.res_f32) load4<float>(p.res, ri, rv); else load4<T>(p.res, ri, rv);
#pragma unroll
          for (int e = 0; e < 4; ++e) v[e] = rv[e] + v[e];
        }
        if constexpr (ACT == 4) {
#pragma unroll
          for (int e = 0; e < 4; ++e) v[e] = fmaxf(v[e], 0.f);
        }
        const size_t oi = (size_t)m * p.out_cstride + p.out_coff + n;
        if (p.out_f32) store4<float>(p.out, oi, v); else store4<T>(p.out, oi, v);
      }
    }
  }
}

template <class T, int BM, int BN, int WM, int MI, int NJ, int NT = 2 * BM, bool MMAJOR = false, class PixFn>
__device__ __forceinline__ void conv_epilogue(const ConvP& p, f32x4 (&acc)[NJ][MI], int n0, uint4* lds, PixFn pix) {
  constexpr int WN = NT / 64 / WM;
  const int tid = threadIdx.x, lane = tid & 63, wave = tid >> 6;
  const int wm0 = (MMAJOR ? wave / WN : wave % WM) * (BM / WM), wn0 = (MMAJOR ? wave % WN : wave / WM) * (BN / WN);
  const int fr = lane & 15, fg = lane >> 4;
  if constexpr (sizeof(T) == 2) {
    constexpr int ROWB = BN * 2;
    constexpr int CPR = BN / 8;
    auto rowswz = [](int row) { if constexpr (CPR <= 16) return row / (16 / CPR); else return row * (CPR / 16); };
    if (!p.res && !p.out_f32 && (p.Cout % 8 == 0) && (p.out_coff % 8 == 0) && (p.out_cstride % 8 == 0)) {
      __syncthreads();
      char* tilep = reinterpret_cast<char*>(lds);
      if (p.act == 1) stage_tile<T, 1, BN, MI, NJ>(p, acc, tilep, n0, wm0, wn0, fr, fg);
      else if (p.act == 2) stage_tile<T, 2, BN, MI, NJ>(p, acc, tilep, n0, wm0, wn0, fr, fg);
      else if (p.act == 3) stage_tile<T, 3, BN, MI, NJ>(p, acc, tilep, n0, wm0, wn0, fr, fg);
      else if (p.act == 4) stage_tile<T, 4, BN, MI, NJ>(p, acc, tilep, n0, wm0, wn0, fr, fg);
      else stage_tile<T, 0, BN, MI, NJ>(p, acc, tilep, n0, wm0, wn0, fr, fg);
      __syncthreads();
      T* outp = reinterpret_cast<T*>(p.out) + p.out_coff + n0;
#pragma unroll
      for (int q = 0; q < (BM * CPR + NT - 1) / NT; ++q) {
        const int idx = tid + NT * q, row = idx / CPR, ch = idx - row * CPR;
        if ((BM * CPR) % NT != 0 && idx >= BM * CPR) break;
        const long m = pix(row);
        if (m >= 0 && n0 + ch * 8 < p.Cout)
          *reinterpret_cast<uint4*>(outp + (size_t)m * p.out_cstride + ch * 8) =
              *reinterpret_cast<const uint4*>(tilep + row * ROWB + (ch ^ (rowswz(row) & (CPR - 1))) * 16);
      }
      return;
    }
  }
  long mrow[MI];
#pragma unroll
  for (int i = 0; i < MI; ++i) mrow[i] = pix(wm0 + i * 16 + fr);
  if (p.act == 1) direct_tile<T, 1, MI, NJ>(p, acc, mrow, n0 + wn0 + fg * 4);
  else if (p.act == 2) direct_tile<T, 2, MI, NJ>(p, acc, mrow, n0 + wn0 + fg * 4);
  else if (p.act == 3) direct_tile<T, 3, MI, NJ>(p, acc, mrow, n0 + wn0 + fg * 4);
  else if (p.act == 4) direct_tile<T, 4, MI, NJ>(p, acc, mrow, n0 + wn0 + fg * 4);
  else direct_tile<T, 0, MI, NJ>(p, acc, mrow, n0 + wn0 + fg * 4);
}

}
```

### clearcam_amd/csrc/dev_bench.hip

```cpp
#include <cmath>
#include "conv_select.h"
#include "yolo_plan.h"

using namespace cc;

extern "C" {

int cc_conv2d_nhwc(int dtype, const void* x_dev, int B, int H, int W, int Cin, const float* w_oihw, const float* bias,
                   int Cout, int k, int stride, int groups, int act, void* out_dev, int force_direct, void* stream) {
  CC_API_BEGIN
  CC_CHECK(x_dev && w_oihw && out_dev && groups >= 1 && Cin % groups == 0 && Cout % groups == 0, "bad argument");
  HostTensor w, b;
  w.shape = {Cout, Cin / groups, k, k};
  w.data.assign(w_oihw, w_oihw + (size_t)Cout * (Cin / groups) * k * k);
  if (bias) { b.shape = {Cout}; b.data.assign(bias, bias + Cout); }
  const int split = dtype == F16S;
  dtype = storage_dtype(dtype);
  PackedConv pc = pack_convs(dtype, {&w}, {bias ? &b : nullptr}, {groups}, 0, split);
  ConvP c{};
  c.s0 = Src{x_dev, H, W, Cin, 0, Cin, 0}; c.s1 = Src{x_dev, 1, 1, 0, 0, 0, 0};
  c.B = B; c.Hin = H; c.Win = W; c.Cin = Cin; c.ks = k; c.stride = stride; c.pad = k / 2;
  c.Ho = (H + 2 * c.pad - k) / stride + 1; c.Wo = (W + 2 * c.pad - k) / stride + 1; c.Cout = Cout; c.Ktot = k * k * Cin * (1 + split); c.Kw = pc.kw;
  c.split = pc.split; c.oscale = pc.oscale;
  c.w = pc.w; c.bias = pc.bias; c.out = out_dev; c.out_cstride = Cout; c.out_coff = 0; c.out_f32 = 0; c.res = nullptr; c.act = act;
  c.variant = force_direct;
  launch_conv(dtype, c, (hipStream_t)stream);
  CC_HIP(hipStreamSynchronize((hipStream_t)stream));
  hipFree(pc.w); hipFree(pc.bias);
  CC_API_END
}

int cc_attn_bench(int dtype, int B, int L, int H, int causal, int abl, int iters, float* ms) {
  CC_API_BEGIN
  CC_CHECK(ms && iters > 0 && (dtype == F16 || dtype == BF16) && B > 0 && L > 0 && H > 0, "bad argument");
  const int D = H * 64;
  const size_t nq = (size_t)B * L * 3 * D, no = (size_t)B * L * D;
  std::vector<float> hx(std::min<size_t>(nq, (size_t)1 << 22));
  uint32_t st = 777u;
  for (auto& v : hx) { st = st * 1664525u + 1013904223u; v = ((st >> 8) & 0xffff) / 65536.0f - 0.5f; }
  std::vector<char> h16(hx.size() * 2);
  convert_f32_to(dtype, hx.data(), h16.data(), hx.size());
  char *qkv = nullptr, *ctx = nullptr;
  CC_HIP(hipMalloc((void**)&qkv, nq * 2 + 256)); CC_HIP(hipMalloc((void**)&ctx, no * 2 + 256));
  for (size_t off = 0; off < nq * 2; off += h16.size()) CC_HIP(hipMemcpy(qkv + off, h16.data(), std::min(h16.size(), nq * 2 - off), hipMemcpyHostToDevice));
  AttnP a{}; a.qkv = qkv; a.ctx = ctx; a.B = B; a.L = L; a.H = H; a.D = D; a.causal = causal; a.scale = 0.125f; a.abl = abl;
  hipStream_t s; CC_HIP(hipStreamCreateWithFlags(&s, hipStreamNonBlocking));
  hipEvent_t e0, e1; CC_HIP(hipEventCreate(&e0)); CC_HIP(hipEventCreate(&e1));
  for (int i = 0; i < 3; ++i) launch_attention(dtype, a, s);
  CC_HIP(hipEventRecord(e0, s));
  for (int i = 0; i < iters; ++i) launch_attention(dtype, a, s);
  CC_HIP(hipEventRecord(e1, s));
  CC_HIP(hipStreamSynchronize(s));
  float t = 0; CC_HIP(hipEventElapsedTime(&t, e0, e1));
  *ms = t / iters;
  hipEventDestroy(e0); hipEventDestroy(e1); hipStreamDestroy(s);
  hipFree(qkv); hipFree(ctx);
  CC_API_END
}

int cc_dev_set(const char* key, int value) {
  CC_API_BEGIN
  CC_CHECK(key, "null key");
  if (std::string(key) == "phase_flags") cc::g_phase_flags_override = value;
  else if (std::string(key) == "stream") cc::g_stream_override = value;
  else if (std::string(key) == "stream_abl") cc::g_stream_abl = value;
  else if (std::string(key) == "stream_flags") cc::g_stream_flags_override = value;
  else if (std::string(key) == "tile64_abl") cc::g_tile64_abl = value;
  else if (std::string(key) == "tile64_w") cc::g_tile64_w_override = value;
  else if (std::string(key) == "index_slab_rows") cc::g_index_slab_rows = value;
  else if (std::string(key) == "index_i8_pass") cc::g_index_i8_pass = value;
  else if (std::string(key) == "index_i8_mfma") cc::g_index_i8_mfma = value;
  else if (std::string(key) == "pool_rows") cc::g_pool_rows_override = value;
  else if (std::string(key) == "csp_tile") cc::g_csp_tile_override = value;
  else if (std::string(key) == "route_log") cc::g_route_log = value ? 1 : 0;
  else throw cc::Error(-22, std::string("cc_dev_set: unknown key ") + key);
  CC_API_END
}

int cc_conv_bench(int dtype, int B, int H, int W, int Cin, int Cout, int k, int stride, int act, int variant, int iters, float* ms) {
  CC_API_BEGIN
  CC_CHECK(ms && iters > 0 && (dtype == F16 || dtype == BF16 || dtype == F16S), "bad argument");
  const int split = dtype == F16S;
  dtype = storage_dtype(dtype);
  HostTensor w, b;
  w.shape = {Cout, Cin, k, k};
  w.data.resize((size_t)Cout * Cin * k * k);
  uint32_t st = 12345u;
  auto rnd = [&]() { st = st * 1664525u + 1013904223u; return ((st >> 8) & 0xffff) / 65536.0f - 0.5f; };
  const float sc = 2.0f / sqrtf((float)Cin * k * k);
  for (auto& v : w.data) v = rnd() * sc;
  b.shape = {Cout}; b.data.assign(Cout, 0.01f);
  PackedConv pc = pack_convs(dtype, {&w}, {&b}, {1}, 0, split);
  const int pad = k / 2, Ho = (H + 2 * pad - k) / stride + 1, Wo = (W + 2 * pad - k) / stride + 1;
  const size_t nin = (size_t)B * H * W * Cin, nout = (size_t)B * Ho * Wo * Cout;
  std::vector<float> hx(std::min<size_t>(nin, (size_t)1 << 24));
  for (auto& v : hx) v = rnd() * 2.0f;
  std::vector<char> hx16(hx.size() * 2);
  convert_f32_to(dtype, hx.data(), hx16.data(), hx.size());
  char *x = nullptr, *out = nullptr;
  CC_HIP(hipMalloc((void**)&x, nin * 2 + 256)); CC_HIP(hipMalloc((void**)&out, nout * 2 + 256));
  for (size_t off = 0; off < nin * 2; off += hx16.size()) CC_HIP(hipMemcpy(x + off, hx16.data(), std::min(hx16.size(), nin * 2 - off), hipMemcpyHostToDevice));
  ConvP c{};
  c.s0 = Src{x, H, W, Cin, 0, Cin, 0}; c.s1 = Src{x, 1, 1, 0, 0, 0, 0};
  c.B = B; c.Hin = H; c.Win = W; c.Cin = Cin; c.ks = k; c.stride = stride; c.pad = pad; c.Ho = Ho; c.Wo = Wo; c.Cout = Cout;
  c.Ktot = k * k * Cin * (1 + split); c.Kw = pc.kw; c.split = pc.split; c.oscale = pc.oscale; c.w = pc.w; c.bias = pc.bias; c.out = out; c.out_cstride = Cout; c.act = act; c.variant = variant;
  hipStream_t s; CC_HIP(hipStreamCreateWithFlags(&s, hipStreamNonBlocking));
  hipEvent_t e0, e1; CC_HIP(hipEventCreate(&e0)); CC_HIP(hipEventCreate(&e1));
  for (int i = 0; i < 3; ++i) launch_conv(dtype, c, s);
  CC_HIP(hipEventRecord(e0, s));
  for (int i = 0; i < iters; ++i) launch_conv(dtype, c, s);
  CC_HIP(hipEventRecord(e1, s));
  CC_HIP(hipStreamSynchronize(s));
  float t = 0; CC_HIP(hipEventElapsedTime(&t, e0, e1));
  *ms = t / iters;
  if (const char* e = getenv("CLEARCAM_BENCH_DUMP")) {
    unsigned long long v[32] = {};
    (void)e;
    CC_HIP(hipMemcpy(v, out + nout * 2, sizeof(v), hipMemcpyDeviceToHost));
    for (int i = 0; i < 32; ++i) fprintf(stderr, "%llu%c", v[i], (i & 3) == 3 ? '\n' : ' ');
  }
  hipEventDestroy(e0); hipEventDestroy(e1); hipStreamDestroy(s);
  hipFree(x); hipFree(out); hipFree(pc.w); hipFree(pc.bias);
  CC_API_END
}

}
```

### include/clearcam_hip.h

```cpp
#ifndef CLEARCAM_HIP_H
#define CLEARCAM_HIP_H
#include <stdint.h>
#ifdef __cplusplus
extern "C" {
#endif

#define CC_DTYPE_F32 0
#define CC_DTYPE_F16 1
#define CC_DTYPE_BF16 2
#define CC_DTYPE_F16S 3
#define CC_DTYPE_F16H 4

#define CC_DTYPE_F16C 5

#define CC_MAX_DET 300

const char* cc_last_error(void);
int cc_version(void);
int cc_device_count(int* n);

typedef struct cc_yolo cc_yolo;

int cc_yolo_create(cc_yolo** h, const char* size, int res, int dtype, int device);
int cc_yolo_load(cc_yolo* h, const char* name, const float* data, const int64_t* shape, int ndim);
int cc_yolo_finalize(cc_yolo* h);
int cc_yolo_calibrate(cc_yolo* h, const void* frames, int B, int H, int W, int frame_f32);
int cc_yolo_calibration_info(cc_yolo* h, int* n_calibrated, int* n_fallback);
int cc_gptq_round_f16(const float* w, int64_t cout, int64_t cin, const double* H, double damp, float* out);
int cc_yolo_detect(cc_yolo* h, const void* frames, int B, int H, int W, int frame_f32,
                   int frames_on_device, float* out, int out_on_device, void* stream);
int cc_yolo_nonfinite(cc_yolo* h, int* count);
int cc_yolo_set_in_flight(cc_yolo* h, int n);
int cc_yolo_submit(cc_yolo* h, const void* frames, int B, int H, int W, int frame_f32, int frames_on_device, float* out,
                   int out_on_device, void* stream, long long* ticket);
int cc_yolo_wait(cc_yolo* h, long long ticket, void* stream);
int cc_yolo_detect_ragged(cc_yolo* h, const void* pixels, const int64_t* offsets, const int32_t* heights, const int32_t* widths, int B,
                          int frame_f32, int pixels_on_device, float* out, int out_on_device, void* stream);
int cc_yolo_submit_ragged(cc_yolo* h, const void* pixels, const int64_t* offsets, const int32_t* heights, const int32_t* widths, int B,
                          int frame_f32, int pixels_on_device, float* out, int out_on_device, void* stream, long long* ticket);
int cc_letterbox_geometry(int H, int W, int res, int* nh, int* nw, int* pad_y, int* pad_x);
int cc_yolo_plans_built(cc_yolo* h, int* n);
int cc_yolo_get_tensor(cc_yolo* h, const char* name, float* out, int64_t* shape, int* ndim);
int cc_yolo_get_tensor_frames(cc_yolo* h, const char* name, int b0, int nb, float* out, int64_t* shape, int* ndim);
int cc_yolo_last_gpu_ms(cc_yolo* h, float* ms);
int cc_yolo_profile(cc_yolo* h, int iters, float* ms, double* alg_macs_per_step, int* n_conv_launches);
int cc_yolo_profile_graph(cc_yolo* h, int iters, int which, float* ms_per_replay);
void cc_yolo_destroy(cc_yolo* h);

int cc_conv2d_nhwc(int dtype, const void* x_dev, int B, int H, int W, int Cin, const float* w_oihw,
                   const float* bias, int Cout, int k, int stride, int groups, int act, void* out_dev,
                   int force_direct, void* stream);
typedef struct {
  int dtype, B, H, W, Cin, Cout, k, stride, groups, act;
  int pad, Ho, Wo;
  int out_f32, out_cstride, out_coff;
  int res_f32, res_cstride, res_coff;
  int variant;
} cc_conv_desc;
int cc_conv2d_ex(const cc_conv_desc* d, const void* x_dev, const float* w_oihw, const float* bias, const float* slope,
                 const void* res_dev, void* out_dev, int* choice, void* stream);
int cc_dev_decode(const float* const* raw_dev, const int* H, const int* W, int B, const float* dfl_w16, float conf, float* det_dev,
                  int* nonfinite, void* stream);
int cc_dev_head_tail(int dtype, int ch, const void* const* bx_dev, const void* const* cl_dev, const float* const* w2, const float* const* b2,
                     const float* const* w3, const float* const* b3, const int* H, const int* W, int B, const float* dfl_w16, float conf,
                     float* det_dev, int* nonfinite, void* stream);
int cc_dev_topk_nms(const float* rows_dev, int B, int A, float iou_thr, const float* geometry, int ragged, float* out_dev, void* stream);
int cc_dev_blaze_post(const float* r8_dev, const float* r16_dev, const float* c8_dev, const float* c16_dev, int B, const float* anchors,
                      float scale, int pad_top, int pad_left, float* out_dev, float* first_dev, int32_t* first_idx_dev, void* stream);
int cc_dev_attention(int dtype, const void* qkv_dev, int B, int L, int H, int causal, float scale, void* ctx_dev, void* stream);
int cc_dev_layernorm(int dtype, const float* in_dev, long long in_row_stride, const int32_t* row_index_dev, const float* w_dev, const float* b_dev,
                     void* out_dev, int out_f32, int rows, int D, void* stream);
int cc_dev_assemble_ln(int dtype, const void* patches_dev, const float* cls_dev, const float* pos_dev, const float* w_dev, const float* b_dev,
                       float* out_dev, int B, int L, int D, void* stream);
int cc_dev_patchify(int dtype, const float* x_dev, void* out_dev, int B, int S, int patch, int Kpad, void* stream);
int cc_dev_embed(const int32_t* tokens, int vocab, const float* table_dev, const float* pos_dev, float* out_dev, int B, int L, int D, void* stream);
int cc_dev_l2norm(float* x_dev, int rows, int D, float eps, void* stream);
typedef struct { const void* ptr; int H, W, cstride, coff, C, shift; } cc_src_desc;
#define CC_DEV_CONV_ADOWN 100
int cc_dev_pool(int dtype, const void* in_dev, int in_cstride, int in_coff, void* out_dev, int out_cstride, int out_coff, int B, int H, int W,
                int C, int Ho, int Wo, int k, int stride, int pad, int mode, int* kernel, void* stream);
int cc_dev_pool_choice(int dtype, const void* in_dev, int in_cstride, int in_coff, void* out_dev, int out_cstride, int out_coff, int B, int H,
                       int W, int C, int Ho, int Wo, int k, int stride, int pad, int mode, int* kernel);
int cc_dev_fuse(int dtype, int n, const void* const* in_dev, const int* H, const int* W, const int* cstride, const int* coff, const int* shift,
                void* out_dev, int out_cstride, int out_coff, int B, int Ho, int Wo, int C, void* stream);
int cc_dev_conv_src(const cc_conv_desc* d, const cc_src_desc* s0, const cc_src_desc* s1, const float* w_oihw, const float* bias, void* out_dev,
                    int* choice, void* stream);
int cc_dev_affine(int dtype, const void* x_dev, void* y_dev, const float* scale_dev, const float* shift_dev, long long n, int C, void* stream);
int cc_dev_face_pre(int dtype, const void* img_dev, int img_f32, void* out_dev, int B, int cpad, void* stream);
#define CC_DEV_CSP_LAYERS 3
int cc_dev_csp(int dtype, int split, int hid, const void* x_dev, int x_cstride, int x_coff, void* out_dev, int out_cstride, int out_coff,
               int B, int H, int W, const float* const* w, const float* const* bias, int variant, int dbg, int* choice, void* stream);
int cc_dev_csp_choice(int dtype, int split, int hid, int B, int H, int W, int variant, int dbg, int* choice);
int cc_dev_stem(int dtype, int split, const void* frames_dev, int frame_f32, const int64_t* offsets, const int32_t* heights, const int32_t* widths,
                int B, int res, int ragged, const float* w_oihw, const float* bias, int Cout, void* out_dev, int out_cstride, int out_coff,
                int* info, void* stream);
int cc_route_log_take(int* records, int cap, int* n);
int cc_conv_bench(int dtype, int B, int H, int W, int Cin, int Cout, int k, int stride, int act, int variant, int iters, float* ms);
int cc_attn_bench(int dtype, int B, int L, int H, int causal, int abl, int iters, float* ms);
int cc_round_weights(int dtype, const float* w, int64_t cout, int64_t cin, int64_t k, float* out);
int cc_dev_set(const char* key, int value);

typedef struct cc_clip cc_clip;
typedef struct {
  int image_size, patch, v_width, v_layers, v_heads, v_mlp;
  int t_ctx, t_vocab, t_width, t_layers, t_heads, t_mlp, embed;
} cc_clip_config;

int cc_clip_create(cc_clip** h, const cc_clip_config* cfg, int dtype, int device);
int cc_clip_load(cc_clip* h, const char* name, const float* data, const int64_t* shape, int ndim);
int cc_clip_finalize(cc_clip* h);
int cc_clip_encode_image(cc_clip* h, const float* x, int B, int x_on_device, float* out, int out_on_device, void* stream);
int cc_clip_encode_text(cc_clip* h, const int32_t* tokens, int B, float* out, int out_on_device, void* stream);
int cc_clip_set_in_flight(cc_clip* h, int n);
int cc_clip_submit_image(cc_clip* h, const float* x, int B, int x_on_device, float* out, int out_on_device, void* stream,
                         long long* ticket);
int cc_clip_wait(cc_clip* h, long long ticket, void* stream);
int cc_clip_last_gpu_ms(cc_clip* h, float* ms);
void cc_clip_destroy(cc_clip* h);

int cc_crop_preprocess(const uint8_t* pixels, const int64_t* offsets, const int32_t* heights, const int32_t* widths,
                       int B, int pixels_on_device, int out_size, float* out_dev, int device, void* stream);

typedef struct cc_face cc_face;
int cc_face_create(cc_face** h, int dtype, int device);
int cc_face_load(cc_face* h, const char* name, const float* data, const int64_t* shape, int ndim);
int cc_face_finalize(cc_face* h);
int cc_face_embed(cc_face* h, const void* faces, int B, int img_f32, int faces_on_device, float* out, int out_on_device, void* stream);
void cc_face_destroy(cc_face* h);

int cc_cv_resize_linear_u8(const uint8_t* src, int H, int W, uint8_t* dst, int dh, int dw, int device);
int cc_cv_warp_affine_u8(const uint8_t* src, int H, int W, const double* M, uint8_t* dst, int dh, int dw, int device);

typedef struct cc_blaze cc_blaze;
int cc_blaze_create(cc_blaze** h, int dtype, int device);
int cc_blaze_load(cc_blaze* h, const char* name, const float* data, const int64_t* shape, int ndim);
int cc_blaze_finalize(cc_blaze* h);
int cc_blaze_detect(cc_blaze* h, const void* img, int H, int W, int img_f32, int img_on_device, float* out, int out_on_device, void* stream);
void cc_blaze_destroy(cc_blaze* h);
int cc_blaze_detect_batch(cc_blaze* h, const void* imgs, int B, int H, int W, int img_f32, int imgs_on_device, float* out, int out_on_device, void* stream);

typedef struct cc_face_align_rec {
  int64_t offset; int32_t h, w;
  int32_t cx1, cy1, cw, ch;
  int32_t out_w, out_h;
  double rot[6], place[6];
} cc_face_align_rec;
int cc_face_locate(cc_blaze* h, const uint8_t* pixels, int64_t pixels_bytes, const int64_t* offsets, const int32_t* heights, const int32_t* widths,
                   int B, int pixels_on_device, float* first, int32_t* first_idx, void* stream);
int cc_face_align(const uint8_t* pixels, int64_t pixels_bytes, int pixels_on_device, const cc_face_align_rec* records, int n,
                  uint8_t* out_dev, int device, void* stream);

typedef struct cc_ocsort cc_ocsort;
int cc_ocsort_create(cc_ocsort** h, int max_age, int min_hits, double iou_threshold, int delta_t, double inertia, int use_byte);
int cc_ocsort_update(cc_ocsort* h, const float* dets, int n, double det_thresh, double* out, int cap, int* n_out);
int cc_ocsort_update_many(cc_ocsort* const* hs, int count, const float* dets, int rows_per, double det_thresh, double* out,
                          int cap_per, int* n_out, int n_threads);
int cc_ocsort_num_tracks(cc_ocsort* h, int* n);
void cc_ocsort_destroy(cc_ocsort* h);

typedef struct cc_index cc_index;
int cc_index_create(cc_index** h, int dim, int64_t capacity, int device);
#define CC_INDEX_I8 8
int cc_index_create_ex(cc_index** h, int dim, int64_t capacity, int device, int storage);
int cc_index_add(cc_index* h, const float* emb, int64_t n, int on_device);
int cc_index_add_grouped(cc_index* h, const float* emb, int64_t n, int on_device, const int32_t* groups);
int cc_index_size(cc_index* h, int64_t* n);
int cc_index_info(cc_index* h, int64_t* capacity, int* storage, int* dim);
int cc_index_scores(cc_index* h, const float* q, int Q, float* scores, int on_device, void* stream);
int cc_index_last_path(cc_index* h, int* path);
int cc_index_search(cc_index* h, const float* q, int Q, int k, int32_t* idx, float* score, int on_device, void* stream);
int cc_index_search_groups(cc_index* h, const float* q, int Q, int k, const uint8_t* allowed, int n_groups, int32_t* idx, float* score,
                           int on_device, void* stream);
int cc_index_add_tracked(cc_index* h, const float* emb, int64_t n, int on_device, const int32_t* groups, const int32_t* tracks);
int cc_index_search_tracks(cc_index* h, const float* q, int Q, int k, const uint8_t* allowed, int n_groups, int32_t* idx, float* score,
                           int on_device, void* stream);
#define CC_RANK_TRACKS 1
int cc_index_rank(cc_index* h, const float* q, int Q, int64_t start, int64_t count, float min_score, int flags,
                  const uint8_t* allowed, int n_groups,
                  int32_t* idx, float* score, int64_t* total, int on_device, void* stream);
#define CC_ROW_NO_TS INT32_MIN
int cc_index_add_described(cc_index* h, const float* emb, int64_t n, int on_device, const int32_t* groups, const int32_t* tracks,
                           const int32_t* ts, const int32_t* cls);
int cc_index_row_info(cc_index* h, int64_t row0, int64_t n, int32_t* ts_out, int32_t* cls_out);
typedef struct { int32_t use_ts, ts_min, ts_max;
                 int32_t use_cls; uint64_t cls_mask[4];  } cc_row_filter;
int cc_index_rank_where(cc_index* h, const float* q, int Q, int64_t start, int64_t count, float min_score, int flags,
                        const uint8_t* allowed, int n_groups, const cc_row_filter* where,
                        int32_t* idx, float* score, int64_t* total, int on_device, void* stream);
int cc_index_timeline(cc_index* h, const float* q, int Q, float min_score, int flags, const uint8_t* allowed, int n_groups,
                      const cc_row_filter* where, int32_t t0, int32_t bin_seconds, int n_bins,
                      uint32_t* counts, int64_t* total, int on_device, void* stream);
int cc_index_fetch_rows(cc_index* h, const int64_t* rows, int n, float* out, int on_device, void* stream);
#define CC_LIKE_MAX_ROWS 64
#define CC_LIKE_EXCLUDE_ROWS  2
#define CC_LIKE_EXCLUDE_TRACK 4
int cc_index_rank_like(cc_index* h, const int64_t* rows, int n_rows, int64_t start, int64_t count, float min_score, int flags,
                       const uint8_t* allowed, int n_groups, const cc_row_filter* where,
                       int32_t* idx, float* score, int64_t* total, int on_device, void* stream);
#define CC_TERMS_MAX 64
#define CC_TERM_RANK    0
#define CC_TERM_REQUIRE 1
#define CC_TERM_REJECT  2
#define CC_COMBINE_MAX 0
#define CC_COMBINE_MIN 1
#define CC_COMBINE_SUM 2
typedef struct { int32_t role; float weight; float cut; } cc_term;
int cc_index_rank_terms(cc_index* h, const float* q, int n_vec, const int64_t* rows, int n_rows,
                        const cc_term* terms, int combine,
                        int64_t start, int64_t count, float min_score, int flags,
                        const uint8_t* allowed, int n_groups, const cc_row_filter* where,
                        int32_t* idx, float* score, int32_t* which, int64_t* total, int on_device, void* stream);
int cc_index_timeline_terms(cc_index* h, const float* q, int n_vec, const int64_t* rows, int n_rows,
                            const cc_term* terms, int combine, float min_score, int flags,
                            const uint8_t* allowed, int n_groups, const cc_row_filter* where,
                            int32_t t0, int32_t bin_seconds, int n_bins,
                            uint32_t* counts, int64_t* total, int on_device, void* stream);
#define CC_DISTINCT_MAX_DEPTH 1024
#define CC_DISTINCT_MAX_Q     64
int cc_index_gram(cc_index* h, const int64_t* rows, int n, float* out, int on_device, void* stream);
int cc_index_distinct(cc_index* h, const int32_t* idx, const float* score, int Q, int depth, float same_at,
                      int64_t start, int64_t count,
                      int32_t* out_idx, float* out_score, int32_t* out_dups, int64_t* total,
                      int on_device, void* stream);
#define CC_DIGEST_MAX_LEADERS 1024
#define CC_DIGEST_BY_COUNT 0
#define CC_DIGEST_BY_FIRST 1
int cc_index_digest(cc_index* h, float same_at, int max_leaders, int order,
                    const uint8_t* allowed, int n_groups, const cc_row_filter* where,
                    int64_t start, int64_t count,
                    int32_t* out_row, int32_t* out_count, int32_t* out_ts_first, int32_t* out_ts_last,
                    int32_t* owner, int64_t* totals, int on_device, void* stream);
#define CC_SIGHT_MAX_OBJECTS 1024
#define CC_SIGHT_MAX_GROUPS  4096
#define CC_SIGHT_SKIP_SELF   1
int cc_index_sightings(cc_index* h, const int64_t* rows, int n, float same_at, int flags,
                       const uint8_t* allowed, int n_groups, const cc_row_filter* where,
                       int32_t* out_count, int32_t* out_best_row, float* out_best_score,
                       uint32_t* out_group_counts, int n_group_counts,
                       int64_t* total, int on_device, void* stream);
int cc_index_remove_rows(cc_index* h, const uint8_t* drop, int64_t n, int64_t* removed);
int cc_index_remove_groups(cc_index* h, const uint8_t* drop, int n_groups, int64_t* removed);
void cc_index_destroy(cc_index* h);

typedef struct cc_watch cc_watch;
#define CC_WATCH_MAX_ALERTS 2048
int cc_watch_create(cc_watch** h, int dim, int device);
int cc_watch_set(cc_watch* h, const float* desc, const float* threshold, const int32_t* group, int A);
int cc_watch_size(cc_watch* h, int* A);
int cc_watch_scores(cc_watch* h, const float* emb, int B, int emb_on_device, float* scores, int on_device, void* stream);
int cc_watch_match(cc_watch* h, const float* emb, int B, int emb_on_device, const int32_t* crop_group, const uint8_t* armed,
                   int32_t* alert, float* score, int on_device, void* stream);
void cc_watch_destroy(cc_watch* h);

#ifdef __cplusplus
}
#endif
#endif
```

Baseline: 6445 frames/s.

## Add register-direct conv epilogue via permuted weight-row loading

Permutes which weight rows each wave loads into LDS so that every lane's MFMA accumulators cover 8 contiguous output channels. The epilogue can then apply bias, activation and residual and write 16-byte stores straight from registers, skipping the LDS staging round-trip. A rule enables this for the persistent phase kernel with Cout<=512 and for 128x128 generic/big tiles that carry a residual, and an override knob plus a getter are added. The cost is extra template instantiations and less coalesced global stores, since each lane writes its own row segment.

```diff
diff --git a/clearcam_amd/_lib.py b/clearcam_amd/_lib.py
--- a/clearcam_amd/_lib.py
+++ b/clearcam_amd/_lib.py
@@ -11,7 +11,7 @@
     "cc_yolo_create", "cc_yolo_load", "cc_yolo_calibrate", "cc_yolo_calibration_info", "cc_gptq_round_f16", "cc_yolo_finalize", "cc_yolo_detect", "cc_yolo_set_in_flight", "cc_yolo_submit", "cc_yolo_wait",
     "cc_yolo_detect_ragged", "cc_yolo_submit_ragged", "cc_letterbox_geometry", "cc_yolo_plans_built",
     "cc_yolo_get_tensor", "cc_yolo_get_tensor_frames", "cc_yolo_nonfinite",
-    "cc_yolo_last_gpu_ms", "cc_yolo_profile", "cc_yolo_profile_graph", "cc_yolo_destroy", "cc_conv2d_nhwc", "cc_conv2d_ex", "cc_route_log_take", "cc_conv_bench", "cc_dev_set", "cc_round_weights", "cc_attn_bench",
+    "cc_yolo_last_gpu_ms", "cc_yolo_profile", "cc_yolo_profile_graph", "cc_yolo_destroy", "cc_conv2d_nhwc", "cc_conv2d_ex", "cc_route_log_take", "cc_conv_bench", "cc_dev_set", "cc_dev_get", "cc_round_weights", "cc_attn_bench",
     "cc_dev_decode", "cc_dev_head_tail", "cc_dev_topk_nms", "cc_dev_blaze_post",
     "cc_dev_pool", "cc_dev_pool_choice", "cc_dev_fuse", "cc_dev_conv_src", "cc_dev_affine", "cc_dev_face_pre",
     "cc_dev_csp", "cc_dev_csp_choice", "cc_dev_stem",
@@ -151,6 +151,7 @@
         "cc_dev_l2norm": [vp, C.c_int, C.c_int, C.c_float, vp],
         "cc_conv_bench": [C.c_int] * 11 + [fp],
         "cc_dev_set": [C.c_char_p, C.c_int],
+        "cc_dev_get": [C.c_char_p, ip],
         "cc_round_weights": [C.c_int, vp, C.c_int64, C.c_int64, C.c_int64, vp],
         "cc_attn_bench": [C.c_int] * 7 + [fp],
         "cc_clip_create": [C.POINTER(vp), C.POINTER(ClipConfig), C.c_int, C.c_int],
diff --git a/clearcam_amd/csrc/conv_mfma.hip b/clearcam_amd/csrc/conv_mfma.hip
--- a/clearcam_amd/csrc/conv_mfma.hip
+++ b/clearcam_amd/csrc/conv_mfma.hip
@@ -69,12 +69,15 @@
       } else { pb[i] = 0; ph0[i] = -(1 << 28); pw0[i] = 0; }
     }
   }
+  constexpr bool REGOK = sizeof(T) == 2 && NJ % 2 == 0;
+  const bool reg = REGOK && a.reg;
+  const int wchunk = reg ? ppos ^ swz_perm<CPRW>(prow) : chunk;
   const char* wcur[WR]; unsigned winc[WR];
 #pragma unroll
   for (int i = 0; i < WR; ++i) {
     const int n = n0 + prow + RPP * i;
     const bool ok = n < p.Cout;
-    wcur[i] = ok ? reinterpret_cast<const char*>(p.w) + ((size_t)n * p.Kw + chunk * E) * sizeof(T) : reinterpret_cast<const char*>(&g_zero16);
+    wcur[i] = ok ? reinterpret_cast<const char*>(p.w) + ((size_t)n * p.Kw + wchunk * E) * sizeof(T) : reinterpret_cast<const char*>(&g_zero16);
     winc[i] = ok ? (unsigned)(BK * sizeof(T)) : 0u;
   }
   int k0 = chunk * E, kc, kr, ks_, vt;
@@ -133,6 +136,12 @@
   const int wm0 = (wave % WM) * (BM / WM), wn0 = (wave / WM) * (BN / WN);
   const int fr = lane & 15, fg = lane >> 4;
   const int nkt = (p.Ktot + BK - 1) / BK;
+  int wrow[NJ], wkey[NJ];
+#pragma unroll
+  for (int j = 0; j < NJ; ++j) {
+    wrow[j] = reg ? wn0 + (j >> 1) * 32 + (j & 1) * 4 + perm_row(fr) : wn0 + j * 16 + fr;
+    wkey[j] = reg ? swz_perm<CPRW>(wrow[j]) : swz<CPRW>(wrow[j]);
+  }
 
   f32x4 acc[NJ][MI];
 #pragma unroll
@@ -163,7 +172,7 @@
 #pragma unroll
       for (int i = 0; i < MI; ++i) { const int row = wm0 + i * 16 + fr; xf[i] = ldsX[row * CPRW + ((h * 4 + fg) ^ swz<CPRW>(row))]; }
 #pragma unroll
-      for (int j = 0; j < NJ; ++j) { const int row = wn0 + j * 16 + fr; wf[j] = ldsW[row * CPRW + ((h * 4 + fg) ^ swz<CPRW>(row))]; }
+      for (int j = 0; j < NJ; ++j) wf[j] = ldsW[wrow[j] * CPRW + ((h * 4 + fg) ^ wkey[j])];
 #pragma unroll
       for (int j = 0; j < NJ; ++j)
 #pragma unroll
@@ -171,10 +180,10 @@
     }
   }
 
-  conv_epilogue<T, BM, BN, WM, MI, NJ, NT>(p, acc, n0, lds, [&](int row) { const int m = m0 + row; return m < M ? (long)m : -1L; });
-}
-
-template <class T, int TS>
+  conv_epilogue<T, BM, BN, WM, MI, NJ, NT>(p, acc, n0, lds, [&](int row) { const int m = m0 + row; return m < M ? (long)m : -1L; }, reg);
+}
+
+template <class T, int TS, bool REG>
 __global__ __launch_bounds__(256, (TS == 256 ? 1 : 2)) void conv_big_kernel(const ConvP p, const ConvAux a) {
   constexpr int BM = TS, BN = TS, NT = 256, WM = 2, WN = 2, MI = BM / WM / 16, NJ = BN / WN / 16;
   constexpr int NF = MI + NJ, MF = MI * NJ, MPG = MF / NF;
@@ -226,7 +235,8 @@
   for (int i = 0; i < WR; ++i) {
     const int n = n0 + prow + RPP * i;
     const bool ok = n < p.Cout;
-    wcur[i] = ok ? reinterpret_cast<const char*>(p.w) + ((size_t)n * p.Kw + chunk * E) * sizeof(T) : reinterpret_cast<const char*>(&g_zero16);
+    const int wchunk = REG ? ppos ^ swz_perm<CPRW>(prow) : chunk;
+    wcur[i] = ok ? reinterpret_cast<const char*>(p.w) + ((size_t)n * p.Kw + wchunk * E) * sizeof(T) : reinterpret_cast<const char*>(&g_zero16);
     winc[i] = ok ? (unsigned)(BK * sizeof(T)) : 0u;
   }
   int k0 = chunk * E, kc, kr, ks_, vt;
@@ -273,6 +283,12 @@
 
   uint4 f0[NF], f1[NF];
   auto frag = [&](int stage, int h, int q) -> uint4 {
+    if constexpr (REG) {
+      if (q >= MI) {
+        const int j = q - MI, srow = wn0 + (j >> 1) * 32 + (j & 1) * 4 + perm_row(fr);
+        return lds[stage * STAGE + (BM + srow) * CPRW + ((h * 4 + fg) ^ swz_perm<CPRW>(srow))];
+      }
+    }
     const int row = (q < MI ? wm0 + q * 16 : BM + wn0 + (q - MI) * 16) + fr;
     const int srow = q < MI ? row : row - BM;
     return lds[stage * STAGE + row * CPRW + ((h * 4 + fg) ^ swz<CPRW>(srow))];
@@ -327,7 +343,7 @@
   for (; kt + 2 < nkt; ++kt) step(kt, std::true_type{}, std::true_type{});
   if (kt + 1 < nkt) { step(kt, std::true_type{}, std::false_type{}); ++kt; }
   step(kt, std::false_type{}, std::false_type{});
-  conv_epilogue<T, BM, BN, WM, MI, NJ, NT>(p, acc, n0, lds, [&](int row) { const int m = m0 + row; return m < M ? (long)m : -1L; });
+  conv_epilogue<T, BM, BN, WM, MI, NJ, NT>(p, acc, n0, lds, [&](int row) { const int m = m0 + row; return m < M ? (long)m : -1L; }, REG);
 }
 
 struct WsAux { float inv_tiles, inv_tx; int tiles, tx, total; };
@@ -450,6 +466,7 @@
 
 std::atomic<int> g_stream_override{-1}, g_phase_flags_override{-1}, g_tile64_w_override{-1}, g_stream_flags_override{-1};
 std::atomic<int> g_stream_abl{0}, g_tile64_abl{0};
+std::atomic<int> g_reg_epilogue_override{-1}, g_reg_epilogue_last{0};
 
 const ConvSwitches& conv_switches() {
   static const ConvSwitches s = [] {
@@ -551,7 +568,33 @@
   return conv_switches().tile64 && (long)B * per_frame >= 256 && per_frame * 256 * 4 <= (long)H * W * 5;
 }
 
+static bool reg_epilogue_legal(int dt, const ConvP& p, const ConvChoice& c) {
+  if (dt == F32 || p.out_f32 || (p.res && p.res_f32)) return false;
+  if (p.Cout % 8 || p.out_coff % 8 || p.out_cstride % 8) return false;
+  if (p.res && (p.res_coff % 8 || p.res_cstride % 8)) return false;
+  switch (c.kernel) {
+    case ConvKernel::Generic: return (c.bn / (c.nth / 64 / c.wm) / 16) % 2 == 0;
+    case ConvKernel::Big: return true;
+    case ConvKernel::Phase: return (c.sched == PHASE_ONE_TILE || c.sched == PHASE_PERSIST) && !(c.flags & (1024 | 0xf000));
+    default: return false;
+  }
+}
+static bool reg_epilogue_rule(int dt, const ConvP& p, const ConvChoice& c) {
+  const int ov = g_reg_epilogue_override.load();
+  if (ov == 0 || !reg_epilogue_legal(dt, p, c)) return false;
+  if (ov > 0) return true;
+  if (c.kernel == ConvKernel::Phase) return c.sched == PHASE_PERSIST && p.Cout <= 512;
+  return p.res != nullptr && c.bm == 128 && c.bn == 128;
+}
+
+static ConvChoice choose_kernel(int dt, const ConvP& p);
 ConvChoice choose_conv(int dt, const ConvP& p) {
+  ConvChoice c = choose_kernel(dt, p);
+  c.reg_epi = reg_epilogue_rule(dt, p, c);
+  return c;
+}
+
+static ConvChoice choose_kernel(int dt, const ConvP& p) {
   const int v = p.variant;
   CC_CHECK(known_variant(v), "conv: ConvP::variant names no kernel");
   ConvChoice c;
@@ -647,12 +690,15 @@
   CC_CHECK(false, "conv_mfma: no such instantiation of the generic kernel");
 }
 
-template <class T, int TS> static void launch_big(const ConvP& p, const ConvAux& a, hipStream_t stream) {
+template <class T, int TS, bool REG> static void launch_big_k(const ConvP& p, const ConvAux& a, hipStream_t stream) {
   constexpr size_t lds = (size_t)2 * (2 * TS) * 8 * 16;
   const int M = p.B * p.Ho * p.Wo;
-  ensure_max_lds(conv_big_kernel<T, TS>, lds);
-  note_launch(TS == 256 ? "conv_big_256" : "conv_big_128", conv_big_kernel<T, TS>, (long)((M + TS - 1) / TS) * a.nt, 256, lds);
-  hipLaunchKernelGGL((conv_big_kernel<T, TS>), dim3(((M + TS - 1) / TS) * a.nt), dim3(256), lds, stream, p, a);
+  ensure_max_lds(conv_big_kernel<T, TS, REG>, lds);
+  note_launch(TS == 256 ? "conv_big_256" : "conv_big_128", conv_big_kernel<T, TS, REG>, (long)((M + TS - 1) / TS) * a.nt, 256, lds);
+  hipLaunchKernelGGL((conv_big_kernel<T, TS, REG>), dim3(((M + TS - 1) / TS) * a.nt), dim3(256), lds, stream, p, a);
+}
+template <class T, int TS> static void launch_big(const ConvP& p, const ConvAux& a, hipStream_t stream) {
+  if (a.reg) launch_big_k<T, TS, true>(p, a, stream); else launch_big_k<T, TS, false>(p, a, stream);
 }
 
 template <class T, int CIN, int COUT> static void launch_ws(const ConvP& p, hipStream_t stream) {
@@ -715,6 +761,8 @@
   a.inv_hw = 1.0f / (float)(p.Ho * p.Wo); a.inv_wo = 1.0f / (float)p.Wo;
   a.is1x1 = c.simple && p.ks == 1 && p.stride == 1 && p.pad == 0 && p.Hin == p.Ho && p.Win == p.Wo;
   a.two = c.two;
+  a.reg = c.reg_epi;
+  g_reg_epilogue_last.store(c.reg_epi, std::memory_order_relaxed);
   switch (c.kernel) {
     case ConvKernel::Direct: launch_conv_direct(dt, p, stream); return;
     case ConvKernel::Stream: launch_conv_stream(dt, p, c, stream); return;
diff --git a/clearcam_amd/csrc/conv_persist.hip b/clearcam_amd/csrc/conv_persist.hip
--- a/clearcam_amd/csrc/conv_persist.hip
+++ b/clearcam_amd/csrc/conv_persist.hip
@@ -22,8 +22,9 @@
   return v;
 }
 
-template <class T, int MM, int ABL = 0>
+template <class T, int MM, int ABL = 0, bool REG = false>
 __global__ __launch_bounds__(512) void conv_persist_kernel(const ConvP p, const ConvAux a) {
+  static_assert(!REG || MM == 0, "the register epilogue is built on the 16x16x32 fragment layout");
   constexpr int BM = 256, BN = 256, NT = 512;
   constexpr int E = 8, CPRW = 8, BK = 64, RPP = NT / CPRW, XR = BM / RPP;
   constexpr int STAGE = (BM + BN) * CPRW;
@@ -99,7 +100,8 @@
       }
       rinfo[i] = ri;
     }
-    wptr = reinterpret_cast<const char*>(p.w) + ((size_t)(n0 + prow) * p.Kw + chunk * E) * sizeof(T);
+    const int wchunk = REG ? (tid_o % CPRW) ^ swz_perm<CPRW>(prow) : chunk;
+    wptr = reinterpret_cast<const char*>(p.w) + ((size_t)(n0 + prow) * p.Kw + wchunk * E) * sizeof(T);
     kc = 0; vt = 0; pt = 0; wt = 0;
     retarget();
   };
@@ -140,9 +142,11 @@
     for (int s = 0; s < NA; ++s) {
       const int ch = MM ? (2 * s + fh) : (4 * s + fh);
       pb[s] = ldsb + (grp * 128 + fr) * 128 + ((ch ^ sw) * 16);
-      wbp[s] = ldsb + (BM + wq * 64 + fr) * 128 + ((ch ^ sw) * 16);
+      const int wfr = REG ? perm_row(fr) : fr, wsw = REG ? swz_perm<CPRW>(wfr) : sw;
+      wbp[s] = ldsb + (BM + wq * 64 + wfr) * 128 + ((ch ^ wsw) * 16);
     }
   }
+  constexpr int WJ = REG ? 4 : 16;
   uint4 pa[8], wb[4], wb1[4];
   f32x4 acc[MM ? 1 : 4][MM ? 1 : 8];
   f32x16 acc32[MM ? 2 : 1][MM ? 4 : 1];
@@ -181,7 +185,7 @@
 #pragma unroll
       for (int kh = 0; kh < 2; ++kh)
 #pragma unroll
-        for (int j = 0; j < 2; ++j) dst[kh * 2 + j] = *reinterpret_cast<const uint4*>(wbp[kh] + so + (ws * 32 + j * 16) * 128);
+        for (int j = 0; j < 2; ++j) dst[kh * 2 + j] = *reinterpret_cast<const uint4*>(wbp[kh] + so + (ws * 32 + j * WJ) * 128);
     } else {
 #pragma unroll
       for (int s = 0; s < 4; ++s) dst[s] = *reinterpret_cast<const uint4*>(wbp[s] + so + (ws * 32) * 128);
@@ -293,6 +297,52 @@
       }
     }
   };
+  auto epilogue_reg = [&](auto act_tag, int em0, int en0, const float4 (&bq)[8], bool full) {
+    constexpr int ACT = decltype(act_tag)::value;
+    if constexpr (MM == 0) {
+      int lane = tid & 63;
+      asm volatile("" : "+v"(lane));
+      const int fr = lane & 15, fg = lane >> 4;
+      const int nb = en0 + wq * 64 + fg * 8;
+      T* outp = reinterpret_cast<T*>(p.out) + p.out_coff + nb;
+      const T* resp = p.res ? reinterpret_cast<const T*>(p.res) + p.res_coff + nb : nullptr;
+      float4 s4[4];
+#pragma unroll
+      for (int k = 0; k < 4; ++k) {
+        if constexpr (ACT == 3) s4[k] = *reinterpret_cast<const float4*>(p.slope + nb + (k >> 1) * 32 + (k & 1) * 4); else s4[k] = make_float4(0.f, 0.f, 0.f, 0.f);
+      }
+#pragma unroll
+      for (int i = 0; i < 8; ++i) {
+        const int m = em0 + grp * 128 + i * 16 + fr;
+        if (full || m < M) {
+#pragma unroll
+          for (int s = 0; s < 2; ++s) {
+            float v[8];
+#pragma unroll
+            for (int h = 0; h < 2; ++h) {
+              const f32x4 av = acc[2 * s + h][i];
+              const float4 b = bq[2 * s + h], sl = s4[2 * s + h];
+              v[4 * h + 0] = act_bias<T, ACT>(osc, av[0], b.x, sl.x); v[4 * h + 1] = act_bias<T, ACT>(osc, av[1], b.y, sl.y);
+              v[4 * h + 2] = act_bias<T, ACT>(osc, av[2], b.z, sl.z); v[4 * h + 3] = act_bias<T, ACT>(osc, av[3], b.w, sl.w);
+            }
+            if (resp) {
+              const uint4 r = *reinterpret_cast<const uint4*>(resp + (size_t)m * p.res_cstride + s * 32);
+              const T* t = reinterpret_cast<const T*>(&r);
+#pragma unroll
+              for (int e = 0; e < 8; ++e) v[e] = to_f32<T>(t[e]) + v[e];
+            }
+            if constexpr (ACT == 4) {
+#pragma unroll
+              for (int e = 0; e < 8; ++e) v[e] = fmaxf(v[e], 0.f);
+            }
+            const uint4 o = make_uint4(pack2<T>(v[0], v[1]), pack2<T>(v[2], v[3]), pack2<T>(v[4], v[5]), pack2<T>(v[6], v[7]));
+            if constexpr (ABL & 32) asm volatile("" :: "v"(o.x), "v"(o.y), "v"(o.z), "v"(o.w));
+            else *reinterpret_cast<uint4*>(outp + (size_t)m * p.out_cstride + s * 32) = o;
+          }
+        }
+      }
+    }
+  };
   auto epilogue32 = [&](auto act_tag, int em0, int en0, const float4 (&bq)[8], bool full) {
     constexpr int ACT = decltype(act_tag)::value;
     int lane = tid & 63;
@@ -397,7 +447,10 @@
 #pragma unroll
     for (int k = 0; k < 8; ++k) bq[k] = make_float4(0.f, 0.f, 0.f, 0.f);
     if (p.bias) {
-      if constexpr (MM == 0) {
+      if constexpr (REG) {
+#pragma unroll
+        for (int k = 0; k < 4; ++k) bq[k] = *reinterpret_cast<const float4*>(p.bias + nb + (k >> 1) * 32 + (lane >> 4) * 8 + (k & 1) * 4);
+      } else if constexpr (MM == 0) {
 #pragma unroll
         for (int j = 0; j < 4; ++j) bq[j] = *reinterpret_cast<const float4*>(p.bias + nb + j * 16 + (lane >> 4) * 4);
       } else {
@@ -407,7 +460,13 @@
     }
   };
   auto epilogue = [&](int em0, int en0, const float4 (&bq)[8], bool full) {
-    if (staged16) {
+    if constexpr (REG) {
+      if (p.act == 1) epilogue_reg(std::integral_constant<int, 1>{}, em0, en0, bq, full);
+      else if (p.act == 2) epilogue_reg(std::integral_constant<int, 2>{}, em0, en0, bq, full);
+      else if (p.act == 3) epilogue_reg(std::integral_constant<int, 3>{}, em0, en0, bq, full);
+      else if (p.act == 4) epilogue_reg(std::integral_constant<int, 4>{}, em0, en0, bq, full);
+      else epilogue_reg(std::integral_constant<int, 0>{}, em0, en0, bq, full);
+    } else if (staged16) {
       if (p.act == 1) epilogue16(std::integral_constant<int, 1>{}, em0, en0, bq, full);
       else if (p.act == 2) epilogue16(std::integral_constant<int, 2>{}, em0, en0, bq, full);
       else if (p.act == 3) epilogue16(std::integral_constant<int, 3>{}, em0, en0, bq, full);
@@ -485,14 +544,14 @@
   return true;
 }
 
-template <class T, int MM, int ABL = 0> static void launch_persist_t(const ConvP& p, const ConvAux& a, int M, hipStream_t stream) {
+template <class T, int MM, int ABL = 0, bool REG = false> static void launch_persist_t(const ConvP& p, const ConvAux& a, int M, hipStream_t stream) {
   constexpr size_t lds = (size_t)2 * 512 * 8 * 16 + 512 * 4 * 16;
-  ensure_max_lds(conv_persist_kernel<T, MM, ABL>, lds);
+  ensure_max_lds(conv_persist_kernel<T, MM, ABL, REG>, lds);
   const int cus = cu_count();
   ConvAux b = a;
   b.ntiles = ((M + 255) / 256) * a.nt;
-  note_launch("conv_persist", conv_persist_kernel<T, MM, ABL>, (long)b.ntiles, 512, lds, std::min(b.ntiles, cus));
-  hipLaunchKernelGGL((conv_persist_kernel<T, MM, ABL>), dim3(std::min(b.ntiles, cus)), dim3(512), lds, stream, p, b);
+  note_launch("conv_persist", conv_persist_kernel<T, MM, ABL, REG>, (long)b.ntiles, 512, lds, std::min(b.ntiles, cus));
+  hipLaunchKernelGGL((conv_persist_kernel<T, MM, ABL, REG>), dim3(std::min(b.ntiles, cus)), dim3(512), lds, stream, p, b);
 }
 
 void launch_conv_persist(int dt, int mm, int abl, const ConvP& p, const ConvAux& a, int M, hipStream_t stream) {
@@ -515,6 +574,7 @@
   if (mm) { if (dt == F16) launch_persist_t<f16_t, 1>(p, a, M, stream); else launch_persist_t<bf16_t, 1>(p, a, M, stream); return; }
 #endif
   (void)abl; (void)mm;
+  if (a.reg) { if (dt == F16) launch_persist_t<f16_t, 0, 0, true>(p, a, M, stream); else launch_persist_t<bf16_t, 0, 0, true>(p, a, M, stream); return; }
   if (dt == F16) launch_persist_t<f16_t, 0>(p, a, M, stream); else launch_persist_t<bf16_t, 0>(p, a, M, stream);
 }
 
diff --git a/clearcam_amd/csrc/conv_phase.hip b/clearcam_amd/csrc/conv_phase.hip
--- a/clearcam_amd/csrc/conv_phase.hip
+++ b/clearcam_amd/csrc/conv_phase.hip
@@ -17,7 +17,7 @@
   asm volatile("s_mov_b32 m0, %2\n\ts_nop 0\n\tbuffer_load_dwordx4 %0, %1, 0 offen lds" : : "v"(voff), "s"(srd), "s"(lds_wave_byte_addr) : "memory", "m0");
 }
 
-template <class T, int SCHED>
+template <class T, int SCHED, bool REG = false>
 __global__ __launch_bounds__(512) void conv_phase_kernel(const ConvP p, const ConvAux a) {
   constexpr int BM = 256, BN = 256, NT = 512, MI = 8, NJ = 4;
   constexpr int E = 8, CPRW = 8, BK = 64, RPP = NT / CPRW, XR = BM / RPP, WR = BN / RPP;
@@ -76,7 +76,8 @@
     }
     rinfo[i] = ri;
   }
-  const char* wptr = reinterpret_cast<const char*>(p.w) + ((size_t)(n0 + prow) * p.Kw + chunk * E) * sizeof(T);
+  const int wchunk = REG ? ppos ^ swz_perm<CPRW>(prow) : chunk;
+  const char* wptr = reinterpret_cast<const char*>(p.w) + ((size_t)(n0 + prow) * p.Kw + wchunk * E) * sizeof(T);
   const size_t wpass = (size_t)RPP * p.Kw * sizeof(T);
   int kc = 0, vt = 0;
   auto retarget = [&]() {
@@ -128,7 +129,9 @@
   const int sw = (fr >> 1) & 7;
   const char* ldsb = reinterpret_cast<const char*>(lds);
   const char* pb[2] = {ldsb + (grp * 128 + fr) * 128 + ((fg ^ sw) * 16), ldsb + (grp * 128 + fr) * 128 + (((4 + fg) ^ sw) * 16)};
-  const char* wbp[2] = {ldsb + (BM + wq * 64 + fr) * 128 + ((fg ^ sw) * 16), ldsb + (BM + wq * 64 + fr) * 128 + (((4 + fg) ^ sw) * 16)};
+  constexpr int WJ = REG ? 4 : 16;
+  const int wfr = REG ? perm_row(fr) : fr, wsw = REG ? swz_perm<CPRW>(wfr) : sw;
+  const char* wbp[2] = {ldsb + (BM + wq * 64 + wfr) * 128 + ((fg ^ wsw) * 16), ldsb + (BM + wq * 64 + wfr) * 128 + (((4 + fg) ^ wsw) * 16)};
   auto read_p = [&](unsigned so, int ps) {
 #pragma unroll
     for (int kh = 0; kh < 2; ++kh)
@@ -141,7 +144,7 @@
     for (int kh = 0; kh < 2; ++kh)
 #pragma unroll
       for (int j = 0; j < 2; ++j)
-        wb[kh * 2 + j] = *reinterpret_cast<const uint4*>(wbp[kh] + so + (ws * 32 + j * 16) * 128);
+        wb[kh * 2 + j] = *reinterpret_cast<const uint4*>(wbp[kh] + so + (ws * 32 + j * WJ) * 128);
   };
   auto mma_w = [&](int ps, int ws, const uint4 (&wv)[4], auto&& mid) {
     __builtin_amdgcn_s_setprio(1);
@@ -161,7 +164,7 @@
     for (int kh = 0; kh < 2; ++kh)
 #pragma unroll
       for (int j = 0; j < 2; ++j)
-        wb1[kh * 2 + j] = *reinterpret_cast<const uint4*>(wbp[kh] + so + (32 + j * 16) * 128);
+        wb1[kh * 2 + j] = *reinterpret_cast<const uint4*>(wbp[kh] + so + (32 + j * WJ) * 128);
   };
   auto end_read = [&]() {
     __builtin_amdgcn_sched_barrier(0);
@@ -245,17 +248,17 @@
   }
   wait_vmcnt<0>();
   if (grp == 0) __builtin_amdgcn_s_barrier();
-  conv_epilogue<T, BM, BN, 2, MI, NJ, NT, true>(p, acc, n0, lds, [&](int row) { const int m = m0 + row; return m < M ? (long)m : -1L; });
+  conv_epilogue<T, BM, BN, 2, MI, NJ, NT, true>(p, acc, n0, lds, [&](int row) { const int m = m0 + row; return m < M ? (long)m : -1L; }, REG);
 }
 
 bool conv_persist_ok(const ConvP& p);
 void launch_conv_persist(int dt, int mm, int abl, const ConvP& p, const ConvAux& a, int M, hipStream_t stream);
-template <class T, int SCHED> static void launch_phase_k(const ConvP& p, const ConvAux& a, hipStream_t stream) {
+template <class T, int SCHED, bool REG = false> static void launch_phase_k(const ConvP& p, const ConvAux& a, hipStream_t stream) {
   constexpr size_t lds = (size_t)2 * 512 * 8 * 16 + 512 * 4 * 16;
   const long tiles = (long)((p.B * p.Ho * p.Wo + 255) / 256) * a.nt;
-  ensure_max_lds(conv_phase_kernel<T, SCHED>, lds);
-  note_launch("conv_phase", conv_phase_kernel<T, SCHED>, tiles, 512, lds);
-  hipLaunchKernelGGL((conv_phase_kernel<T, SCHED>), dim3(tiles), dim3(512), lds, stream, p, a);
+  ensure_max_lds(conv_phase_kernel<T, SCHED, REG>, lds);
+  note_launch("conv_phase", conv_phase_kernel<T, SCHED, REG>, tiles, 512, lds);
+  hipLaunchKernelGGL((conv_phase_kernel<T, SCHED, REG>), dim3(tiles), dim3(512), lds, stream, p, a);
 }
 
 template <class T> static void launch_phase(const ConvP& p, const ConvAux& a, const ConvChoice& c, hipStream_t stream) {
@@ -264,7 +267,7 @@
   switch (c.sched) {
     case PHASE_PERSIST: launch_conv_persist(TypeTag<T>::dt, (c.flags & 1024) ? 1 : 0, (c.flags >> 12) & 15, p, b, p.B * p.Ho * p.Wo, stream); break;
     case PHASE_BUFFER: launch_phase_k<T, 2>(p, b, stream); break;
-    case PHASE_ONE_TILE: launch_phase_k<T, 1>(p, b, stream); break;
+    case PHASE_ONE_TILE: if (b.reg) launch_phase_k<T, 1, true>(p, b, stream); else launch_phase_k<T, 1>(p, b, stream); break;
     default: launch_phase_k<T, 0>(p, b, stream);
   }
 }
diff --git a/clearcam_amd/csrc/conv_select.h b/clearcam_amd/csrc/conv_select.h
--- a/clearcam_amd/csrc/conv_select.h
+++ b/clearcam_amd/csrc/conv_select.h
@@ -38,6 +38,7 @@
   int flags = 0;
   int tile64_w = 32;
   int cin = 0, cout = 0;
+  bool reg_epi = false;
 };
 
 ConvChoice choose_conv(int dt, const ConvP& p);
@@ -61,5 +62,6 @@
 
 extern std::atomic<int> g_stream_override, g_phase_flags_override, g_tile64_w_override, g_stream_flags_override;
 extern std::atomic<int> g_stream_abl, g_tile64_abl;
+extern std::atomic<int> g_reg_epilogue_override, g_reg_epilogue_last;
 
 }
diff --git a/clearcam_amd/csrc/conv_tile.h b/clearcam_amd/csrc/conv_tile.h
--- a/clearcam_amd/csrc/conv_tile.h
+++ b/clearcam_amd/csrc/conv_tile.h
@@ -16,6 +16,7 @@
   unsigned x_bytes, w_bytes;
   int ntiles;
   int two;
+  int reg;
 };
 
 __device__ __forceinline__ float out_scale(const ConvP& p) { return p.split ? p.oscale : 1.0f; }
@@ -79,6 +80,11 @@
   if constexpr (CPRW == 8) return (row >> 1) & 7;
   else return (-(row >> 2)) & 3;
 }
+__device__ __forceinline__ int perm_row(int fr) { return (fr >> 2) * 8 + (fr & 3); }
+template <int CPRW> __device__ __forceinline__ int swz_perm(int row) {
+  if constexpr (CPRW == 8) return ((row >> 1) & 1) | (((row >> 3) & 3) << 1);
+  else return (row >> 3) & 3;
+}
 template <int N> __device__ __forceinline__ void wait_vmcnt() { asm volatile("s_waitcnt vmcnt(%0)" ::"n"(N) : "memory"); }
 
 template <class T, int ACT, int BN, int MI, int NJ>
@@ -145,12 +151,72 @@
   }
 }
 
+template <class T, int ACT, int MI, int NJ>
+__device__ __forceinline__ void reg_tile(const ConvP& p, const f32x4 (&acc)[NJ][MI], const long (&mrow)[MI], int nbase) {
+  static_assert(sizeof(T) == 2 && NJ % 2 == 0, "16-bit storage, whole fragment pairs");
+  const float osc = out_scale(p);
+#pragma unroll
+  for (int s = 0; s < NJ / 2; ++s) {
+    const int n = nbase + s * 32;
+    const bool nok = n + 8 <= p.Cout;
+    float bv[8] = {0.f, 0.f, 0.f, 0.f, 0.f, 0.f, 0.f, 0.f}, sv[8] = {0.f, 0.f, 0.f, 0.f, 0.f, 0.f, 0.f, 0.f};
+    if (p.bias && nok) {
+      const float4 b0 = *reinterpret_cast<const float4*>(p.bias + n), b1 = *reinterpret_cast<const float4*>(p.bias + n + 4);
+      bv[0] = b0.x; bv[1] = b0.y; bv[2] = b0.z; bv[3] = b0.w; bv[4] = b1.x; bv[5] = b1.y; bv[6] = b1.z; bv[7] = b1.w;
+    }
+    if constexpr (ACT == 3) {
+      if (nok) {
+        const float4 s0 = *reinterpret_cast<const float4*>(p.slope + n), s1 = *reinterpret_cast<const float4*>(p.slope + n + 4);
+        sv[0] = s0.x; sv[1] = s0.y; sv[2] = s0.z; sv[3] = s0.w; sv[4] = s1.x; sv[5] = s1.y; sv[6] = s1.z; sv[7] = s1.w;
+      }
+    }
+#pragma unroll
+    for (int i = 0; i < MI; ++i) {
+      const long m = mrow[i];
+      if (nok && m >= 0) {
+        float v[8];
+#pragma unroll
+        for (int e = 0; e < 8; ++e) {
+          v[e] = activate<T, ACT>(__builtin_fmaf(acc[2 * s + (e >> 2)][i][e & 3], osc, bv[e]));
+          if constexpr (ACT == 3) v[e] = v[e] > 0.f ? v[e] : sv[e] * v[e];
+        }
+        if (p.res) {
+          const uint4 r = *reinterpret_cast<const uint4*>(reinterpret_cast<const T*>(p.res) + (size_t)m * p.res_cstride + p.res_coff + n);
+          const T* t = reinterpret_cast<const T*>(&r);
+#pragma unroll
+          for (int e = 0; e < 8; ++e) v[e] = to_f32<T>(t[e]) + v[e];
+        }
+        if constexpr (ACT == 4) {
+#pragma unroll
+          for (int e = 0; e < 8; ++e) v[e] = fmaxf(v[e], 0.f);
+        }
+        *reinterpret_cast<uint4*>(reinterpret_cast<T*>(p.out) + (size_t)m * p.out_cstride + p.out_coff + n) =
+            make_uint4(pack2<T>(v[0], v[1]), pack2<T>(v[2], v[3]), pack2<T>(v[4], v[5]), pack2<T>(v[6], v[7]));
+      }
+    }
+  }
+}
+
 template <class T, int BM, int BN, int WM, int MI, int NJ, int NT = 2 * BM, bool MMAJOR = false, class PixFn>
-__device__ __forceinline__ void conv_epilogue(const ConvP& p, f32x4 (&acc)[NJ][MI], int n0, uint4* lds, PixFn pix) {
+__device__ __forceinline__ void conv_epilogue(const ConvP& p, f32x4 (&acc)[NJ][MI], int n0, uint4* lds, PixFn pix, bool reg = false) {
   constexpr int WN = NT / 64 / WM;
   const int tid = threadIdx.x, lane = tid & 63, wave = tid >> 6;
   const int wm0 = (MMAJOR ? wave / WN : wave % WM) * (BM / WM), wn0 = (MMAJOR ? wave % WN : wave / WM) * (BN / WN);
   const int fr = lane & 15, fg = lane >> 4;
+  if constexpr (sizeof(T) == 2 && NJ % 2 == 0) {
+    if (reg) {
+      long mrow[MI];
+#pragma unroll
+      for (int i = 0; i < MI; ++i) mrow[i] = pix(wm0 + i * 16 + fr);
+      const int nbase = n0 + wn0 + fg * 8;
+      if (p.act == 1) reg_tile<T, 1, MI, NJ>(p, acc, mrow, nbase);
+      else if (p.act == 2) reg_tile<T, 2, MI, NJ>(p, acc, mrow, nbase);
+      else if (p.act == 3) reg_tile<T, 3, MI, NJ>(p, acc, mrow, nbase);
+      else if (p.act == 4) reg_tile<T, 4, MI, NJ>(p, acc, mrow, nbase);
+      else reg_tile<T, 0, MI, NJ>(p, acc, mrow, nbase);
+      return;
+    }
+  }
   if constexpr (sizeof(T) == 2) {
     constexpr int ROWB = BN * 2;
     constexpr int CPR = BN / 8;
diff --git a/clearcam_amd/csrc/dev_bench.hip b/clearcam_amd/csrc/dev_bench.hip
--- a/clearcam_amd/csrc/dev_bench.hip
+++ b/clearcam_amd/csrc/dev_bench.hip
@@ -73,7 +73,16 @@
   else if (std::string(key) == "pool_rows") cc::g_pool_rows_override = value;
   else if (std::string(key) == "csp_tile") cc::g_csp_tile_override = value;
   else if (std::string(key) == "route_log") cc::g_route_log = value ? 1 : 0;
+  else if (std::string(key) == "reg_epilogue") cc::g_reg_epilogue_override = value;
   else throw cc::Error(-22, std::string("cc_dev_set: unknown key ") + key);
+  CC_API_END
+}
+
+int cc_dev_get(const char* key, int* value) {
+  CC_API_BEGIN
+  CC_CHECK(key && value, "null argument");
+  if (std::string(key) == "reg_epilogue_last") *value = cc::g_reg_epilogue_last.load();
+  else throw cc::Error(-22, std::string("cc_dev_get: unknown key ") + key);
   CC_API_END
 }
 
diff --git a/include/clearcam_hip.h b/include/clearcam_hip.h
--- a/include/clearcam_hip.h
+++ b/include/clearcam_hip.h
@@ -99,6 +99,7 @@
 int cc_attn_bench(int dtype, int B, int L, int H, int causal, int abl, int iters, float* ms);
 int cc_round_weights(int dtype, const float* w, int64_t cout, int64_t cin, int64_t k, float* out);
 int cc_dev_set(const char* key, int value);
+int cc_dev_get(const char* key, int* value);
 
 typedef struct cc_clip cc_clip;
 typedef struct {
```

After: 6484 frames/s, median of 6. No clear change (+0.6%).
